# stdstu12/YUME

Hardware: NVIDIA H100
Metric: latent_frames_per_sec (higher is better)
Workload: dtype bf16

## Files before the change

include/yume_b200.h:

```cpp
#ifndef YUME_B200_H_
#define YUME_B200_H_

#ifdef __cplusplus
extern "C" {
#endif

#define YB_OK 0
#define YB_ERR_ARG (-1)
#define YB_ERR_SHAPE (-2)
#define YB_ERR_ALIGNMENT (-3)
#define YB_ERR_NO_DRIVER (-4)
#define YB_ERR_TENSORMAP (-5)
#define YB_ERR_LAUNCH (-6)

int yb_abi_version(void);

#define YB_EPI_BF16 0
#define YB_EPI_GELU_BF16 1
#define YB_EPI_F32 2
#define YB_EPI_GATE_RES 3
#define YB_EPI_RES_BF16 5
#define YB_EPI_GELU_ERF_BF16 4

typedef struct yb_gemm_args {
  unsigned int struct_bytes;
  int cta_pair;
  const void* A;
  const void* B;
  const void* bias;
  void* out;
  const void* gate;
  const void* tok_idx;
  long long lda, ldb, ldo, gate_ld;
  int M, N, K;
  int epilogue;
  int block_n;
  int n_split;
  long long split_stride;
  int a_split;
  long long a_split_stride;
  const void* res;
  long long res_ld;
  int split_k;
  void* ws;
  long long ws_bytes;
} yb_gemm_args;
int yb_gemm_bf16(const yb_gemm_args* args, void* stream);
long long yb_gemm_workspace_bytes(int M, int N, int K, int epilogue, int cta_pair, int split_k);
int yb_gemm_splitk_plan(int tiles, int num_kb, int clusters, int split_k, int* out3);
int yb_gemm_plan(int M, int N, int sms, int* out4);

typedef struct yb_conv3d_args {
  unsigned int struct_bytes;
  int cta_pair;
  const void* xpad;
  const void* w;
  const void* bias;
  void* out;
  const void* res;
  long long ldo, res_ld;
  int T, H, W, Cp, Cout;
  int epilogue;
  int kt, kh, kw;
  int oob_zero_pad;
  int out_t_mul, out_t_add;
  int fuse_w;
  int stride_t, stride_hw;
} yb_conv3d_args;
int yb_conv3d_causal(const yb_conv3d_args* args, void* stream);
int yb_conv3d_plan(int T, int H, int W, int Cout, int kw, int fuse_w, int* out4);

int yb_ln_modulate(const void* x, long long ldx, void* out, long long ldo, int out_f32, const void* scale,
                   const void* shift, long long mod_ld, const void* tok_idx, const void* weight, const void* lnbias,
                   int L, int C, float eps, void* stream);

int yb_rmsnorm_rope(void* qk, long long ld, const void* weight, const void* rope, int rope_len, int L, int C, int D,
                    float eps, void* stream);
int yb_rmsnorm_rope_pieces(void* qk, long long ld, int piece_cols, long long piece_stride, const void* weight,
                           const void* rope, int rope_len, int L, int C, int D, float eps, void* stream);

int yb_qk_norm_rope(void* q, void* k, long long ld, int piece_cols, long long piece_stride, const void* wq, const void* wk,
                    const void* rope, int rope_len, int L, int C, int D, float eps, void* stream);

int yb_attention(const void* q, long long ldq, const void* k, long long ldk, const void* v, long long ldv, void* out,
                 long long ldo, int Lq, int Lk, int heads, float scale, int flags, void* stream);
int yb_attention_ex(const void* q, long long ldq, const void* k, long long ldk, const void* v, long long ldv, void* out,
                    long long ldo, int Lq, int Lk, int heads, float scale, int flags, void* ws, long long ws_bytes,
                    void* trace, void* stream);
#define YB_ATT_P_SMEM 1
#define YB_ATT_EMU_SHIFT 2
#define YB_ATT_ACCUMULATE 2
#define YB_ATT_SPLIT_SHIFT 4
int yb_attention_plan(int Lq, int Lk, int heads, int sms, int flags, int* out4);
long long yb_attention_workspace_bytes(int Lq, int Lk, int heads, int sms, int flags);
int yb_debug_force_split(int ns);
int yb_sp_scatter_qkv(const void* qkv, long long ld, const void* wq, const void* wk, const void* rope, int rope_len,
                      int L, int C, int D, float eps, void* const* peers, int world, int rank, int Lp, void* stream);
int yb_gemm_sp_qkv(const void* A, long long lda, const void* W, const void* bias, int Lp_rows, int C, int K, void* const* peers,
                   int world, int rank, int Lp, void* sums, void* stream);
int yb_sp_bcast_sums(void* local_sums, void* const* peer_tables, int world, int rank, int Lp, void* stream);
int yb_sp_post_norm_rope(void* buf, const void* sums, const void* wq, const void* wk, const void* rope, int rope_len, int L,
                         int Wh, int C, int D, float eps, void* stream);
int yb_attention_sp(const void* q, long long ldq, const void* k, long long ldk, const void* v, long long ldv,
                    void* const* out_peers, long long ldo, int Lq, int Lk, int heads, float scale, int world, int rank,
                    int Lp, int flags, void* ws, long long ws_bytes, void* stream);

int yb_patchify(const void* x, long long sc, long long sf, long long sh, long long sw, void* out, long long ldo,
                int Cin, int F, int H, int W, int ph, int pw, void* stream);

int yb_unpatchify(const void* y, long long ldy, void* out, int Cout, int F, int Hp, int Wp, int ph, int pw,
                  void* stream);

int yb_bcast_add(const void* a, const void* b, void* out, int R1, int R2, int n, void* stream);

int yb_sinusoidal(const void* t, void* out, int n, int dim, void* stream);

int yb_linear_f32_small(const void* in, const void* W, const void* bias, void* out, int M, int N, int K, int silu_in,
                        void* stream);

int yb_linear_f32(const void* in, long long ldi, const void* W, const void* bias, void* out, long long ldo, int M,
                  int N, int K, void* stream);

int yb_gn_stats(const void* x, long long ld, void* stats, long long N, int C, int G, void* stream);
int yb_vae_pad_act(const void* x, long long ldx, int Ts, int Hs, int Ws, int C, void* out, int Cp, int pad, int ft, int fh,
                   int fw, const void* stats, const void* gamma, const void* beta, int G, float eps, int silu,
                   void* stream);
int yb_masked_softmax(const void* S, long long ldS, void* P, long long ldP, int L, int hw, void* stream);
int yb_nchw_to_nhwc_bf16(const void* x, void* out, long long N, int Cn, int ldo, void* stream);
int yb_nhwc_to_nchw_f32(const void* x, long long ldx, void* out, long long N, int Cn, void* stream);
int yb_nhwc_to_nchw_f32_clamp(const void* x, long long ldx, void* out, long long N, int Cn, float lo, float hi, void* stream);
int yb_blend(const void* a, void* b, long long outer, int ea, int eb, int ext, long long inner, void* stream);

int yb_vae_assemble_tiles(const void* const* tile_ptrs, const int* th, const int* tw, const int* tlen, const int* tf0, int nt,
                          int ni, int nj, int C, int F, int H, int W, int row_limit, int blend_extent, int t_limit,
                          int t_blend_extent, void* out, void* stream);

int yb_vae_rms_act(const void* x, long long ldx, void* out, const void* gamma, int T, int Hs, int Ws, int C, int Cp, int up,
                   int silu, void* stream);
int yb_vae_dupup_add(void* main_, const void* x, int Ts, int Hs, int Ws, int in_c, int out_c, int ft, int fs, void* stream);
int yb_vae_unpatchify2_clamp(const void* y, long long ldy, void* out, int T, int H, int W, void* stream);
int yb_vae_avgdown_add(void* main_, const void* x, int T, int H, int W, int in_c, int out_c, int ft, int fs, void* stream);
int yb_vae_patchify2_bf16(const void* video, void* out, long long ldo, int T, int H, int W, void* stream);

int yb_umma_probe(const void* A, const void* B, void* D, int mode, void* stream);

#ifdef __cplusplus
}
#endif
#endif
```

yume_b200/_lib.py:

```python
from __future__ import annotations

import ctypes as C
from pathlib import Path

_LIB_PATH = Path(__file__).resolve().parent / "csrc" / "libyume_b200.so"

YB_EPI_BF16, YB_EPI_GELU_BF16, YB_EPI_F32, YB_EPI_GATE_RES, YB_EPI_GELU_ERF_BF16, YB_EPI_RES_BF16 = 0, 1, 2, 3, 4, 5
YB_ATT_P_SMEM, YB_ATT_ACCUMULATE = 1, 2
ABI_VERSION = 4
YB_ATT_EMU_SHIFT, YB_ATT_SPLIT_SHIFT = 2, 4

_ERRORS = {
    -1: "YB_ERR_ARG (null pointer / bad enum / non-positive size)",
    -2: "YB_ERR_SHAPE (shape not supported by the kernel)",
    -3: "YB_ERR_ALIGNMENT (pointer or stride not 16-byte aligned)",
    -4: "YB_ERR_NO_DRIVER (cuTensorMapEncodeTiled unavailable: no CUDA driver)",
    -5: "YB_ERR_TENSORMAP (driver rejected a TMA descriptor)",
    -6: "YB_ERR_LAUNCH (kernel launch failed)",
}


class YumeB200Error(RuntimeError):
    pass


class GemmArgs(C.Structure):

    _fields_ = [
        ("struct_bytes", C.c_uint), ("cta_pair", C.c_int),
        ("A", C.c_void_p), ("B", C.c_void_p), ("bias", C.c_void_p), ("out", C.c_void_p),
        ("gate", C.c_void_p), ("tok_idx", C.c_void_p),
        ("lda", C.c_longlong), ("ldb", C.c_longlong), ("ldo", C.c_longlong), ("gate_ld", C.c_longlong),
        ("M", C.c_int), ("N", C.c_int), ("K", C.c_int), ("epilogue", C.c_int), ("block_n", C.c_int),
        ("n_split", C.c_int), ("split_stride", C.c_longlong), ("a_split", C.c_int), ("a_split_stride", C.c_longlong),
        ("res", C.c_void_p), ("res_ld", C.c_longlong),
        ("split_k", C.c_int), ("ws", C.c_void_p), ("ws_bytes", C.c_longlong),
    ]


class Conv3dArgs(C.Structure):

    _fields_ = [
        ("struct_bytes", C.c_uint), ("cta_pair", C.c_int),
        ("xpad", C.c_void_p), ("w", C.c_void_p), ("bias", C.c_void_p), ("out", C.c_void_p), ("res", C.c_void_p),
        ("ldo", C.c_longlong), ("res_ld", C.c_longlong),
        ("T", C.c_int), ("H", C.c_int), ("W", C.c_int), ("Cp", C.c_int), ("Cout", C.c_int), ("epilogue", C.c_int),
        ("kt", C.c_int), ("kh", C.c_int), ("kw", C.c_int), ("oob_zero_pad", C.c_int), ("out_t_mul", C.c_int),
        ("out_t_add", C.c_int), ("fuse_w", C.c_int), ("stride_t", C.c_int), ("stride_hw", C.c_int),
    ]


_vp, _ll, _i, _f = C.c_void_p, C.c_longlong, C.c_int, C.c_float
SIGNATURES = {
    "yb_abi_version": (_i, []),
    "yb_gemm_bf16": (_i, [C.POINTER(GemmArgs), _vp]),
    "yb_conv3d_causal": (_i, [C.POINTER(Conv3dArgs), _vp]),
    "yb_gn_stats": (_i, [_vp, _ll, _vp, _ll, _i, _i, _vp]),
    "yb_vae_pad_act": (_i, [_vp, _ll, _i, _i, _i, _i, _vp, _i, _i, _i, _i, _i, _vp, _vp, _vp, _i, _f, _i, _vp]),
    "yb_masked_softmax": (_i, [_vp, _ll, _vp, _ll, _i, _i, _vp]),
    "yb_nchw_to_nhwc_bf16": (_i, [_vp, _vp, _ll, _i, _i, _vp]),
    "yb_nhwc_to_nchw_f32": (_i, [_vp, _ll, _vp, _ll, _i, _vp]),
    "yb_gemm_plan": (_i, [_i, _i, _i, C.POINTER(C.c_int)]),
    "yb_gemm_workspace_bytes": (_ll, [_i, _i, _i, _i, _i, _i]),
    "yb_gemm_splitk_plan": (_i, [_i, _i, _i, _i, C.POINTER(C.c_int)]),
    "yb_conv3d_plan": (_i, [_i, _i, _i, _i, _i, _i, C.POINTER(C.c_int)]),
    "yb_attention_plan": (_i, [_i, _i, _i, _i, _i, C.POINTER(C.c_int)]),
    "yb_nhwc_to_nchw_f32_clamp": (_i, [_vp, _ll, _vp, _ll, _i, C.c_float, C.c_float, _vp]),
    "yb_blend": (_i, [_vp, _vp, _ll, _i, _i, _i, _ll, _vp]),
    "yb_vae_assemble_tiles": (_i, [_vp, _vp, _vp, _vp, _vp, _i, _i, _i, _i, _i, _i, _i, _i, _i, _i, _i, _vp, _vp]),
    "yb_vae_rms_act": (_i, [_vp, _ll, _vp, _vp, _i, _i, _i, _i, _i, _i, _i, _vp]),
    "yb_vae_dupup_add": (_i, [_vp, _vp, _i, _i, _i, _i, _i, _i, _i, _vp]),
    "yb_vae_unpatchify2_clamp": (_i, [_vp, _ll, _vp, _i, _i, _i, _vp]),
    "yb_vae_avgdown_add": (_i, [_vp, _vp, _i, _i, _i, _i, _i, _i, _i, _vp]),
    "yb_vae_patchify2_bf16": (_i, [_vp, _vp, _ll, _i, _i, _i, _vp]),
    "yb_ln_modulate": (_i, [_vp, _ll, _vp, _ll, _i, _vp, _vp, _ll, _vp, _vp, _vp, _i, _i, _f, _vp]),
    "yb_rmsnorm_rope": (_i, [_vp, _ll, _vp, _vp, _i, _i, _i, _i, _f, _vp]),
    "yb_rmsnorm_rope_pieces": (_i, [_vp, _ll, _i, _ll, _vp, _vp, _i, _i, _i, _i, _f, _vp]),
    "yb_qk_norm_rope": (_i, [_vp, _vp, _ll, _i, _ll, _vp, _vp, _vp, _i, _i, _i, _i, _f, _vp]),
    "yb_attention": (_i, [_vp, _ll, _vp, _ll, _vp, _ll, _vp, _ll, _i, _i, _i, _f, _i, _vp]),
    "yb_attention_ex": (_i, [_vp, _ll, _vp, _ll, _vp, _ll, _vp, _ll, _i, _i, _i, _f, _i, _vp, _ll, _vp, _vp]),
    "yb_attention_workspace_bytes": (_ll, [_i, _i, _i, _i, _i]),
    "yb_debug_force_split": (_i, [_i]),
    "yb_sp_scatter_qkv": (_i, [_vp, _ll, _vp, _vp, _vp, _i, _i, _i, _i, _f, C.POINTER(C.c_void_p), _i, _i, _i, _vp]),
    "yb_gemm_sp_qkv": (_i, [_vp, _ll, _vp, _vp, _i, _i, _i, C.POINTER(C.c_void_p), _i, _i, _i, _vp, _vp]),
    "yb_sp_bcast_sums": (_i, [_vp, C.POINTER(C.c_void_p), _i, _i, _i, _vp]),
    "yb_sp_post_norm_rope": (_i, [_vp, _vp, _vp, _vp, _vp, _i, _i, _i, _i, _i, _f, _vp]),
    "yb_attention_sp": (_i, [_vp, _ll, _vp, _ll, _vp, _ll, C.POINTER(C.c_void_p), _ll, _i, _i, _i, _f, _i, _i, _i, _i, _vp, _ll,
                             _vp]),
    "yb_patchify": (_i, [_vp, _ll, _ll, _ll, _ll, _vp, _ll, _i, _i, _i, _i, _i, _i, _vp]),
    "yb_bcast_add": (_i, [_vp, _vp, _vp, _i, _i, _i, _vp]),
    "yb_unpatchify": (_i, [_vp, _ll, _vp, _i, _i, _i, _i, _i, _i, _vp]),
    "yb_sinusoidal": (_i, [_vp, _vp, _i, _i, _vp]),
    "yb_linear_f32_small": (_i, [_vp, _vp, _vp, _vp, _i, _i, _i, _i, _vp]),
    "yb_linear_f32": (_i, [_vp, _ll, _vp, _vp, _vp, _ll, _i, _i, _i, _vp]),
    "yb_umma_probe": (_i, [_vp, _vp, _vp, _i, _vp]),
}

CLIP_SIGNATURES = {
    "yb_resize_bicubic_normalize": (_i, [_vp, _ll, _ll, _ll, _i, _i, _i, _vp, _i, _vp, _vp, _vp]),
}

T5_SIGNATURES = {
    "yb_t5_attention": (_i, [_vp, _ll, _vp, _ll, _vp, _ll, _vp, _ll, _i, _i, _i, _vp, _vp, _vp]),
    "yb_t5_rmsnorm": (_i, [_vp, _ll, _vp, _ll, _i, _vp, _i, _i, _f, _vp]),
    "yb_t5_geglu": (_i, [_vp, _ll, _vp, _ll, _i, _i, _vp]),
}

STREAM_SIGNATURES = {
    "yb_conv3d_causal_hist": (_i, [C.POINTER(Conv3dArgs), _i, _vp]),
    "yb_vae_dupup_add_cont": (_i, [_vp, _vp, _i, _i, _i, _i, _i, _i, _i, _vp]),
    "yb_vae_unpatchify2_clamp_win": (_i, [_vp, _ll, _vp, _ll, _i, _i, _i, _vp]),
    "yb_nhwc_to_nchw_f32_clamp_win": (_i, [_vp, _ll, _vp, _ll, _ll, _i, _f, _f, _vp]),
    "yb_vae_patchify2_bf16_win": (_i, [_vp, _ll, _vp, _ll, _i, _i, _i, _vp]),
    "yb_nchw_to_nhwc_bf16_win": (_i, [_vp, _ll, _vp, _ll, _i, _i, _vp]),
}

YB_EPI_GELU_FP8 = 8


class GemmFp8Args(C.Structure):

    _fields_ = [
        ("struct_bytes", C.c_uint), ("M", C.c_int), ("N", C.c_int), ("K", C.c_int),
        ("A", C.c_void_p), ("a_scale", C.c_void_p), ("B", C.c_void_p), ("b_scale", C.c_void_p), ("bias", C.c_void_p),
        ("out", C.c_void_p), ("out_scale", C.c_void_p), ("gate", C.c_void_p), ("tok_idx", C.c_void_p),
        ("lda", C.c_longlong), ("lds", C.c_longlong), ("ldb", C.c_longlong), ("ldo", C.c_longlong), ("ldos", C.c_longlong),
        ("gate_ld", C.c_longlong), ("epilogue", C.c_int), ("block_n", C.c_int),
    ]


FP8_SIGNATURES = {
    "yb_gemm_fp8": (_i, [C.POINTER(GemmFp8Args), _vp]),
    "yb_ln_modulate_fp8": (_i, [_vp, _ll, _vp, _ll, _vp, _ll, _vp, _vp, _ll, _vp, _vp, _vp, _i, _i, _f, _vp]),
    "yb_quant_rows_fp8": (_i, [_vp, _ll, _vp, _ll, _vp, _ll, _i, _i, _vp]),
}

FP8_ATTN_SIGNATURES = {
    "yb_quant_vt_fp8": (_i, [_vp, _ll, _vp, _vp, _i, _i, _vp]),
    "yb_attention_fp8": (_i, [_vp, _ll, _vp, _ll, _vp, _ll, _vp, _vp, _vp, _ll, _i, _i, _i, _f, _i, _vp, _ll, _vp]),
}

class Conv3dFp8Args(C.Structure):

    _fields_ = [
        ("struct_bytes", C.c_uint), ("x", C.c_void_p), ("x_scale", C.c_void_p), ("w", C.c_void_p), ("w_scale", C.c_void_p),
        ("bias", C.c_void_p), ("out", C.c_void_p), ("res", C.c_void_p), ("ldo", C.c_longlong), ("res_ld", C.c_longlong),
        ("T", C.c_int), ("H", C.c_int), ("W", C.c_int), ("Cp", C.c_int), ("Cout", C.c_int),
        ("kt", C.c_int), ("kh", C.c_int), ("kw", C.c_int), ("t_hist", C.c_int), ("epilogue", C.c_int),
    ]


FP8_VAE_SIGNATURES = {
    "yb_conv3d_fp8": (_i, [C.POINTER(Conv3dFp8Args), _vp]),
    "yb_vae_rms_act_fp8": (_i, [_vp, _ll, _vp, _vp, _vp, _i, _i, _i, _i, _i, _i, _i, _vp]),
}

_lib = None


def lib_path() -> Path:
    return _LIB_PATH


def load():
    global _lib
    if _lib is not None:
        return _lib
    if not _LIB_PATH.exists():
        raise YumeB200Error(
            f"{_LIB_PATH} is missing: build it with `python -m yume_b200.build` (or __graft_entry__.build()). "
            "yume_b200 has no fallback path.")
    lib = C.CDLL(str(_LIB_PATH))
    if lib.yb_abi_version() != ABI_VERSION:
        raise YumeB200Error(f"{_LIB_PATH} has ABI version {lib.yb_abi_version()}, this binding expects {ABI_VERSION}: rebuild it "
                            "(python -m yume_b200.build --force)")
    for name, (res, args) in {**SIGNATURES, **CLIP_SIGNATURES, **T5_SIGNATURES, **STREAM_SIGNATURES,
                              **FP8_SIGNATURES, **FP8_ATTN_SIGNATURES, **FP8_VAE_SIGNATURES}.items():
        fn = getattr(lib, name)
        fn.restype = res
        fn.argtypes = args
    _lib = lib
    return lib


def check(rc: int, what: str) -> None:
    if rc != 0:
        raise YumeB200Error(f"{what} failed: {_ERRORS.get(rc, rc)}")
```

yume_b200/csrc/gemm.cu:

```cuda
#include "yb_host.h"
#include "../../include/yume_b200_stream.h"
#include "yb_ptx.cuh"

namespace yb {

constexpr int GEMM_BLOCK_M = 128;
constexpr int GEMM_BLOCK_K = 64;
constexpr int GEMM_THREADS = 384;
constexpr int GEMM_GROUP_N = 8;
constexpr int GEMM_MAX_STAGES = 8;
constexpr int GEMM_SMEM_BYTES = 227 * 1024;
constexpr int GEMM_A_BYTES = GEMM_BLOCK_M * GEMM_BLOCK_K * 2;
constexpr int GEMM_EPI_STAGE_BYTES = 8 * 16 * 36 * 4;
constexpr int GEMM_EPI_BOX_BYTES = 64 * 128;
constexpr int GEMM_EPI_TMA_BYTES = 2 * 2 * GEMM_EPI_BOX_BYTES;

struct GemmParams {
  int M, N, K;
  const float* bias;
  void* out;
  long long ldo;
  const float* gate;
  long long gate_ld;
  const int* tok_idx;
  int a_split;
  int n_split;
  long long split_stride;
  const __nv_bfloat16* res;
  long long res_ld;
  int conv, cin_chunks;
  int TW, TH, TT, tiles_w, tiles_h;
  int cT, cH, cW;
  int kh, kw;
  int off_t, off_h, off_w;
  int out_t_mul, out_t_add;
  int st_t, st_h, st_w;
  int num_m_tiles, num_n_tiles;
  int block_n, stages;
  int sk_full, sk_ns, sk_per;
  float* sk_ws;
  int tma_out;
  __nv_bfloat16* sp_peers[8];
  float* sp_sums;
  int sp_rank, sp_Lp, sp_Wh, sp_C;
};
constexpr int YB_EPI_SP_QKV = 6;

constexpr int CONVW_ROWS = GEMM_BLOCK_M + 2;
constexpr int CONVW_A_SLAB = 17 * 1024;
constexpr int CONVW_A_STAGES = 4;

__host__ __device__ constexpr int gemm_b_bytes(int block_n) { return ((block_n + 63) / 64) * 64 * GEMM_BLOCK_K * 2; }
__host__ __device__ constexpr int gemm_stage_bytes(int block_n, int convw) { return (convw ? 0 : GEMM_A_BYTES) + gemm_b_bytes(block_n); }
__host__ __device__ constexpr int gemm_a_ring_bytes(int convw) { return convw ? CONVW_A_STAGES * CONVW_A_SLAB : 0; }
__host__ __device__ constexpr bool gemm_has_tma_epilogue(int epi, int convw, int cluster) {
  return cluster == 1 && !convw && (epi == YB_EPI_BF16 || epi == YB_EPI_GELU_BF16 || epi == YB_EPI_GELU_ERF_BF16 ||
                                    epi == YB_EPI_F32 || epi == YB_EPI_GATE_RES);
}
__host__ __device__ constexpr bool gemm_tma_epilogue_only(int epi, int convw, int cluster) {
  return gemm_has_tma_epilogue(epi, convw, cluster) && epi != YB_EPI_BF16 && epi != YB_EPI_F32;
}
__host__ __device__ constexpr int gemm_epi_bytes(bool tma) { return tma ? GEMM_EPI_TMA_BYTES : GEMM_EPI_STAGE_BYTES; }
static int gemm_stages(int block_n, int convw, int epi_bytes) {
  const int s = (GEMM_SMEM_BYTES - 1024 - 256 - epi_bytes - gemm_a_ring_bytes(convw)) / gemm_stage_bytes(block_n, convw);
  return s > GEMM_MAX_STAGES ? GEMM_MAX_STAGES : s;
}

__device__ __forceinline__ void tile_coords(int tile, int num_m_tiles, int num_n_tiles, int& m_tile, int& n_tile) {
  const int per_group = GEMM_GROUP_N * num_m_tiles;
  const int g = tile / per_group;
  const int r = tile - g * per_group;
  const int n_first = g * GEMM_GROUP_N;
  const int n_in_group = min(GEMM_GROUP_N, num_n_tiles - n_first);
  m_tile = r / n_in_group;
  n_tile = n_first + (r - m_tile * n_in_group);
}

template <int EPI>
__device__ __forceinline__ void epilogue_rows16(const GemmParams& p, int col0, int my_row, int my_tok, const float* stage, int lane,
                                                float* sq) {
  constexpr bool kBf16Out = (EPI == YB_EPI_BF16 || EPI == YB_EPI_GELU_BF16 || EPI == YB_EPI_GELU_ERF_BF16 ||
                             EPI == YB_EPI_RES_BF16 || EPI == YB_EPI_SP_QKV);
  if (col0 >= p.N) return;
  if (kBf16Out) {
    const int cq = (lane & 3) * 8;
    float b[8] = {0.f, 0.f, 0.f, 0.f, 0.f, 0.f, 0.f, 0.f};
    if (p.bias) {
      const float4 b0 = __ldg(reinterpret_cast<const float4*>(p.bias + col0 + cq));
      const float4 b1 = __ldg(reinterpret_cast<const float4*>(p.bias + col0 + cq + 4));
      b[0] = b0.x; b[1] = b0.y; b[2] = b0.z; b[3] = b0.w; b[4] = b1.x; b[5] = b1.y; b[6] = b1.z; b[7] = b1.w;
    }
    long long col_off = col0 + cq;
    if (p.n_split > 0) col_off = static_cast<long long>(col0 / p.n_split) * p.split_stride + (col0 % p.n_split) + cq;
    __nv_bfloat16* obase = reinterpret_cast<__nv_bfloat16*>(p.out) + col_off;
    long long ld = p.ldo;
    if (EPI == YB_EPI_SP_QKV) {
      const int part = col0 / p.sp_C, cin = col0 - part * p.sp_C;
      const int peer = cin / p.sp_Wh;
      ld = 3LL * p.sp_Wh;
      obase = p.sp_peers[peer] + static_cast<long long>(p.sp_rank) * p.sp_Lp * ld + part * p.sp_Wh + (cin - peer * p.sp_Wh) + cq;
    }
    uint4 resv[2];
    if (EPI == YB_EPI_RES_BF16) {
#pragma unroll
      for (int it = 0; it < 2; ++it) {
        const int rowi = __shfl_sync(0xffffffffu, my_row, it * 8 + (lane >> 2));
        resv[it] = make_uint4(0u, 0u, 0u, 0u);
        if (rowi >= 0) resv[it] = *reinterpret_cast<const uint4*>(p.res + static_cast<long long>(rowi) * p.res_ld + col0 + cq);
      }
    }
#pragma unroll
    for (int it = 0; it < 2; ++it) {
      const int rr = it * 8 + (lane >> 2);
      const int rowi = __shfl_sync(0xffffffffu, my_row, rr);
      const float4 a0 = *reinterpret_cast<const float4*>(stage + rr * 36 + cq);
      const float4 a1 = *reinterpret_cast<const float4*>(stage + rr * 36 + cq + 4);
      float v[8] = {a0.x + b[0], a0.y + b[1], a0.z + b[2], a0.w + b[3], a1.x + b[4], a1.y + b[5], a1.z + b[6], a1.w + b[7]};
      if (EPI == YB_EPI_GELU_BF16) {
#pragma unroll
        for (int i = 0; i < 8; ++i) v[i] = gelu_tanh(v[i]);
      }
      if (EPI == YB_EPI_GELU_ERF_BF16) {
#pragma unroll
        for (int i = 0; i < 8; ++i) v[i] = 0.5f * v[i] * (1.0f + erff(v[i] * 0.7071067811865476f));
      }
      if (EPI == YB_EPI_RES_BF16) {
        const __nv_bfloat162* rh = reinterpret_cast<const __nv_bfloat162*>(&resv[it]);
#pragma unroll
        for (int i = 0; i < 4; ++i) {
          const float2 f = __bfloat1622float2(rh[i]);
          v[2 * i] += f.x;
          v[2 * i + 1] += f.y;
        }
      }
      if (rowi >= 0) {
        uint4 w;
        w.x = pack_bf16x2(v[0], v[1]);
        w.y = pack_bf16x2(v[2], v[3]);
        w.z = pack_bf16x2(v[4], v[5]);
        w.w = pack_bf16x2(v[6], v[7]);
        *reinterpret_cast<uint4*>(obase + static_cast<long long>(rowi) * ld) = w;
        if (EPI == YB_EPI_SP_QKV) {
          const __nv_bfloat162* wh = reinterpret_cast<const __nv_bfloat162*>(&w);
          float acc = 0.f;
#pragma unroll
          for (int i = 0; i < 4; ++i) {
            const float2 f = __bfloat1622float2(wh[i]);
            acc += f.x * f.x + f.y * f.y;
          }
          sq[it] += acc;
        }
      }
    }
  } else {
    const int cq = (lane & 7) * 4;
    float4 b = make_float4(0.f, 0.f, 0.f, 0.f);
    if (p.bias) b = __ldg(reinterpret_cast<const float4*>(p.bias + col0 + cq));
    float* obase = reinterpret_cast<float*>(p.out) + col0 + cq;
    float4 xv[4], gv[4];
    int rowv[4];
#pragma unroll
    for (int it = 0; it < 4; ++it) {
      const int rr = it * 4 + (lane >> 3);
      const int tok = __shfl_sync(0xffffffffu, my_tok, rr);
      rowv[it] = __shfl_sync(0xffffffffu, my_row, rr);
      xv[it] = make_float4(0.f, 0.f, 0.f, 0.f);
      gv[it] = make_float4(1.f, 1.f, 1.f, 1.f);
      if (EPI == YB_EPI_GATE_RES && rowv[it] >= 0) {
        xv[it] = *reinterpret_cast<const float4*>(obase + static_cast<long long>(rowv[it]) * p.ldo);
        if (p.gate) gv[it] = __ldg(reinterpret_cast<const float4*>(p.gate + static_cast<long long>(tok) * p.gate_ld + col0 + cq));
      }
    }
#pragma unroll
    for (int it = 0; it < 4; ++it) {
      const int rr = it * 4 + (lane >> 3);
      float4 a = *reinterpret_cast<const float4*>(stage + rr * 36 + cq);
      a.x += b.x; a.y += b.y; a.z += b.z; a.w += b.w;
      if (rowv[it] >= 0) {
        float4* o4 = reinterpret_cast<float4*>(obase + static_cast<long long>(rowv[it]) * p.ldo);
        if (EPI == YB_EPI_F32) {
          *o4 = a;
        } else {
          float4 x = xv[it];
          x.x += a.x * gv[it].x; x.y += a.y * gv[it].y; x.z += a.z * gv[it].z; x.w += a.w * gv[it].w;
          *o4 = x;
        }
      }
    }
  }
}

template <int EPI, int NM>
__device__ __forceinline__ void epilogue_tma(const GemmParams& p, const CUtensorMap* tmO, const float (&acc)[128], uint8_t* bufs,
                                             int row0, int col0, int wg, int wtid, uint32_t& nbox) {
  constexpr bool kF32 = (EPI == YB_EPI_F32 || EPI == YB_EPI_GATE_RES);
  constexpr int BOX_COLS = kF32 ? 32 : 64;
  constexpr int GROUPS = BOX_COLS / 8;
  if (row0 >= p.M) return;
  const int lane = wtid & 31;
  const int r = (wtid >> 5) * 16 + (lane >> 2);
  const int sw = lane >> 2, c2 = 2 * (lane & 3);
  const int ncols = min(NM, p.N - col0);
  const float* g_lo = nullptr;
  const float* g_hi = nullptr;
  if (EPI == YB_EPI_GATE_RES && p.gate != nullptr) {
    int t_lo = 0, t_hi = 0;
    if (p.tok_idx != nullptr) {
      if (row0 + r < p.M) t_lo = p.tok_idx[row0 + r];
      if (row0 + r + 8 < p.M) t_hi = p.tok_idx[row0 + r + 8];
    }
    g_lo = p.gate + static_cast<long long>(t_lo) * p.gate_ld;
    g_hi = p.gate + static_cast<long long>(t_hi) * p.gate_ld;
  }
#pragma unroll
  for (int s = 0; s < NM / BOX_COLS; ++s) {
    if (s * BOX_COLS < ncols) {
      uint8_t* buf = bufs + (nbox & 1) * GEMM_EPI_BOX_BYTES;
      if (wtid == 0) bulk_wait_read<1>();
      named_bar_sync(1 + wg, 128);
#pragma unroll
      for (int j = 0; j < GROUPS; ++j) {
        const int g = s * GROUPS + j;
        const int col = col0 + s * BOX_COLS + 8 * j + c2;
        float2 b = make_float2(0.f, 0.f);
        const bool in = s * BOX_COLS + 8 * j < ncols;
        if (p.bias && in) b = __ldg(reinterpret_cast<const float2*>(p.bias + col));
        float2 lo = make_float2(acc[4 * g] + b.x, acc[4 * g + 1] + b.y);
        float2 hi = make_float2(acc[4 * g + 2] + b.x, acc[4 * g + 3] + b.y);
        if (EPI == YB_EPI_GELU_BF16) {
          lo = make_float2(gelu_tanh(lo.x), gelu_tanh(lo.y));
          hi = make_float2(gelu_tanh(hi.x), gelu_tanh(hi.y));
        }
        if (EPI == YB_EPI_GELU_ERF_BF16) {
          auto ge = [](float v) { return 0.5f * v * (1.0f + erff(v * 0.7071067811865476f)); };
          lo = make_float2(ge(lo.x), ge(lo.y));
          hi = make_float2(ge(hi.x), ge(hi.y));
        }
        if (EPI == YB_EPI_GATE_RES && g_lo != nullptr && in) {
          const float2 gl = __ldg(reinterpret_cast<const float2*>(g_lo + col));
          const float2 gh = __ldg(reinterpret_cast<const float2*>(g_hi + col));
          lo = make_float2(lo.x * gl.x, lo.y * gl.y);
          hi = make_float2(hi.x * gh.x, hi.y * gh.y);
        }
        if (kF32) {
          const int off = (((2 * j + ((lane & 3) >> 1)) ^ sw) << 4) + 8 * (lane & 1);
          *reinterpret_cast<float2*>(buf + r * 128 + off) = lo;
          *reinterpret_cast<float2*>(buf + (r + 8) * 128 + off) = hi;
        } else {
          const int off = ((j ^ sw) << 4) + 4 * (lane & 3);
          *reinterpret_cast<uint32_t*>(buf + r * 128 + off) = pack_bf16x2(lo.x, lo.y);
          *reinterpret_cast<uint32_t*>(buf + (r + 8) * 128 + off) = pack_bf16x2(hi.x, hi.y);
        }
      }
      fence_proxy_async_smem();
      named_bar_sync(1 + wg, 128);
      if (wtid == 0) {
        if (EPI == YB_EPI_GATE_RES) tma_reduce_add_2d(tmO, buf, col0 + s * BOX_COLS, row0);
        else tma_store_2d(tmO, buf, col0 + s * BOX_COLS, row0);
        bulk_commit();
      }
      ++nbox;
    }
  }
}

template <int NM>
__device__ __forceinline__ void gemm_mma_k64(float (&acc)[128], uint32_t sa, uint32_t sb, int block_n, bool zero_first) {
  const uint64_t ad0 = make_smem_desc_sw128(sa, 16, 1024), bd0 = make_smem_desc_sw128(sb, 16, 1024);
  const int nb64 = (block_n + 63) >> 6;
#pragma unroll
  for (int k = 0; k < GEMM_BLOCK_K / 16; ++k) {
    const uint64_t ad = ad0 + 2 * k, bd = bd0 + 2 * k;
    const uint32_t accum = (zero_first && k == 0) ? 0u : 1u;
    if (NM == 256) {
      wgmma_ss_n256<0>(acc, ad, bd, accum);
    } else if (NM == 128) {
      wgmma_ss_n128<0>(acc, ad, bd, accum);
    } else {
      wgmma_ss_n64<0>(acc, ad, bd, accum);
      if (nb64 > 1) wgmma_ss_n64<32>(acc, ad, bd + (8192 >> 4), accum);
      if (nb64 > 2) wgmma_ss_n64<64>(acc, ad, bd + (16384 >> 4), accum);
      if (nb64 > 3) wgmma_ss_n64<96>(acc, ad, bd + (24576 >> 4), accum);
    }
  }
}

template <int CLUSTER>
__device__ __forceinline__ void release_slot(uint64_t* bar, int lane) {
  __syncwarp();
  if (lane == 0) {
    if (CLUSTER == 1) {
      mbar_arrive(bar);
    } else {
      mbar_arrive_cluster(bar, 0);
      mbar_arrive_cluster(bar, 1);
    }
  }
}

template <int EPI, int CONVW, int CLUSTER, int NM>
__global__ void __launch_bounds__(GEMM_THREADS, 1)
gemm_kernel(const __grid_constant__ CUtensorMap tmA, const __grid_constant__ CUtensorMap tmB, const __grid_constant__ CUtensorMap tmO,
            const GemmParams p) {
  static_assert(!(CONVW && CLUSTER != 1), "the kw-fused conv runs on single CTAs");
  constexpr bool kTmaEpi = gemm_has_tma_epilogue(EPI, CONVW, CLUSTER);
  const bool tma_out = gemm_tma_epilogue_only(EPI, CONVW, CLUSTER) || (kTmaEpi && p.tma_out);
  extern __shared__ uint8_t smem_raw[];
  uint8_t* smem = reinterpret_cast<uint8_t*>((reinterpret_cast<uintptr_t>(smem_raw) + 1023) & ~uintptr_t(1023));
  const int block_n = p.block_n, stages = p.stages;
  const int stage_bytes = gemm_stage_bytes(block_n, CONVW);
  uint8_t* a_ring = smem + stages * stage_bytes;
  float* epi = reinterpret_cast<float*>(a_ring + gemm_a_ring_bytes(CONVW));
  uint64_t* full_bar = reinterpret_cast<uint64_t*>(reinterpret_cast<uint8_t*>(epi) + gemm_epi_bytes(kTmaEpi));
  uint64_t* empty_bar = full_bar + GEMM_MAX_STAGES;
  uint64_t* a_full = empty_bar + GEMM_MAX_STAGES;
  uint64_t* a_empty = a_full + CONVW_A_STAGES;

  const int warp = threadIdx.x >> 5, lane = threadIdx.x & 31;
  const int rank = CLUSTER == 2 ? static_cast<int>(cluster_ctarank()) : 0;
  const int tile_first = blockIdx.x / CLUSTER, tile_step = gridDim.x / CLUSTER;
  const int num_tiles = p.num_m_tiles * p.num_n_tiles;
  const int num_kb = (p.K + GEMM_BLOCK_K - 1) / GEMM_BLOCK_K;
  const int num_work = p.sk_full + (num_tiles - p.sk_full) * p.sk_ns;
  auto decode_work = [&](int w, int& tile, int& kb0, int& kb1, int& part) {
    tile = w; kb0 = 0; kb1 = num_kb; part = -1;
    if (w >= p.sk_full) {
      const int u = w - p.sk_full;
      tile = p.sk_full + u / p.sk_ns;
      kb0 = (u % p.sk_ns) * p.sk_per;
      kb1 = min(num_kb, kb0 + p.sk_per);
      part = u;
    }
  };
  auto conv_box = [&](int mt, int& it, int& ih, int& iw) {
    const int per_t = p.tiles_h * p.tiles_w;
    it = mt / per_t;
    const int rem = mt - it * per_t;
    ih = rem / p.tiles_w;
    iw = rem - ih * p.tiles_w;
  };

  if (threadIdx.x == 0) {
    tma_prefetch_desc(&tmA);
    tma_prefetch_desc(&tmB);
    if (tma_out) tma_prefetch_desc(&tmO);
    for (int i = 0; i < stages; ++i) {
      mbar_init(&full_bar[i], 1);
      mbar_init(&empty_bar[i], 8 * CLUSTER);
    }
    for (int i = 0; i < (CONVW ? CONVW_A_STAGES : 0); ++i) {
      mbar_init(&a_full[i], 1);
      mbar_init(&a_empty[i], 8);
    }
    fence_barrier_init();
  }
  __syncthreads();
  if (CLUSTER > 1) cluster_sync_all();

  if (warp < 4) {
    setmaxnreg_dec<40>();
    if (warp == 0 && lane == 0) {
      int stage = 0, a_stage = 0;
      uint32_t phase = 0, a_phase = 0;
      for (int w = tile_first; w < num_work; w += tile_step) {
        int tile, kb0, kb1, part, m_tile, n_tile;
        decode_work(w, tile, kb0, kb1, part);
        tile_coords(tile, p.num_m_tiles, p.num_n_tiles, m_tile, n_tile);
        if (CONVW) {
          int it, ih, iw;
          conv_box(m_tile, it, ih, iw);
          const int groups = num_kb / 3;
          for (int g = 0; g < groups; ++g) {
            const int tdh = g / p.cin_chunks, cc = g - tdh * p.cin_chunks;
            const int dt = tdh / p.kh, dh = tdh - dt * p.kh;
            mbar_wait(&a_empty[a_stage], a_phase ^ 1);
            mbar_arrive_expect_tx(&a_full[a_stage], CONVW_ROWS * GEMM_BLOCK_K * 2);
            tma_load_4d(a_ring + a_stage * CONVW_A_SLAB, &tmA, &a_full[a_stage], cc * GEMM_BLOCK_K, iw * GEMM_BLOCK_M - p.off_w,
                        ih + dh - p.off_h, it + dt - p.off_t);
            if (++a_stage == CONVW_A_STAGES) {
              a_stage = 0;
              a_phase ^= 1;
            }
#pragma unroll 1
            for (int dw = 0; dw < 3; ++dw) {
              mbar_wait(&empty_bar[stage], phase ^ 1);
              mbar_arrive_expect_tx(&full_bar[stage], block_n * GEMM_BLOCK_K * 2);
              tma_load_2d(smem + stage * stage_bytes, &tmB, &full_bar[stage], ((tdh * 3 + dw) * p.cin_chunks + cc) * GEMM_BLOCK_K,
                          n_tile * block_n);
              if (++stage == stages) {
                stage = 0;
                phase ^= 1;
              }
            }
          }
          continue;
        }
        for (int kb = kb0; kb < kb1; ++kb) {
          if (CLUSTER > 1) mbar_wait_cluster(&empty_bar[stage], phase ^ 1);
          else mbar_wait(&empty_bar[stage], phase ^ 1);
          uint8_t* sa = smem + stage * stage_bytes;
          uint8_t* sb = sa + GEMM_A_BYTES;
          mbar_arrive_expect_tx(&full_bar[stage], GEMM_A_BYTES + block_n * GEMM_BLOCK_K * 2);
          const int kcol = kb * GEMM_BLOCK_K;
          const int mt = m_tile * CLUSTER + rank;
          if (p.conv) {
            const int tap = kb / p.cin_chunks, cc = kb - tap * p.cin_chunks;
            const int dt = tap / (p.kh * p.kw), dh = (tap / p.kw) % p.kh, dw = tap % p.kw;
            int it, ih, iw;
            conv_box(mt, it, ih, iw);
            tma_load_4d(sa, &tmA, &full_bar[stage], cc * GEMM_BLOCK_K, iw * p.TW * p.st_w + dw - p.off_w,
                        ih * p.TH * p.st_h + dh - p.off_h, it * p.TT * p.st_t + dt - p.off_t);
          } else {
            const int chunk = kcol / p.a_split;
            tma_load_3d(sa, &tmA, &full_bar[stage], kcol - chunk * p.a_split, mt * GEMM_BLOCK_M, chunk);
          }
          if (CLUSTER == 1) {
            tma_load_2d(sb, &tmB, &full_bar[stage], kcol, n_tile * block_n);
          } else {
            const int half = block_n / 2;
            tma_load_2d_multicast(sb + rank * half * GEMM_BLOCK_K * 2, &tmB, &full_bar[stage], kcol, n_tile * block_n + rank * half,
                                  static_cast<uint16_t>(3));
          }
          if (++stage == stages) {
            stage = 0;
            phase ^= 1;
          }
        }
      }
    }
  } else {
    setmaxnreg_inc<232>();
    const int wg = (warp >> 2) - 1;
    const int r0 = wg * 64 + (warp & 3) * 16;
    float* stage_buf = epi + (warp - 4) * (16 * 36);
    uint8_t* box_bufs = reinterpret_cast<uint8_t*>(epi) + wg * 2 * GEMM_EPI_BOX_BYTES;
    uint32_t nbox = 0;
    int stage = 0, a_stage = 0;
    uint32_t phase = 0, a_phase = 0;
    float acc[128];
#pragma unroll
    for (int i = 0; i < 128; ++i) acc[i] = 0.f;
    for (int w = tile_first; w < num_work; w += tile_step) {
      int tile, kb0, kb1, part, m_tile, n_tile;
      decode_work(w, tile, kb0, kb1, part);
      tile_coords(tile, p.num_m_tiles, p.num_n_tiles, m_tile, n_tile);
      const int mt = m_tile * CLUSTER + rank;
      int my_row = -1;
      if (!tma_out) {
        const int r = r0 + (lane & 15);
        if (p.conv) {
          int it, ih, iw;
          conv_box(mt, it, ih, iw);
          const int tw = r % p.TW, th = (r / p.TW) % p.TH, tt = r / (p.TW * p.TH);
          const int t = it * p.TT + tt, h = ih * p.TH + th, ww = iw * p.TW + tw;
          my_row = (t < p.cT && h < p.cH && ww < p.cW) ? ((t * p.out_t_mul + p.out_t_add) * p.cH + h) * p.cW + ww : -1;
        } else {
          const int row = mt * GEMM_BLOCK_M + r;
          my_row = row < p.M ? row : -1;
        }
      }
      if (EPI == YB_EPI_GATE_RES && part < 0 && my_row >= 0 && lane < 16) {
        const char* xrow = reinterpret_cast<const char*>(reinterpret_cast<const float*>(p.out) +
                                                         static_cast<long long>(my_row) * p.ldo + n_tile * block_n);
        const int ncols = min(block_n, p.N - n_tile * block_n);
        for (int b = 0; b < ncols * 4; b += 128) asm volatile("prefetch.global.L2 [%0];" ::"l"(xrow + b));
      }
      int prev = -1;
      if (CONVW) {
        int prev_a = -1;
        const int groups = num_kb / 3;
        for (int g = 0; g < groups; ++g) {
          mbar_wait(&a_full[a_stage], a_phase);
          const uint32_t sa = smem_u32(a_ring + a_stage * CONVW_A_SLAB) + wg * 64 * 128;
#pragma unroll 1
          for (int dw = 0; dw < 3; ++dw) {
            mbar_wait(&full_bar[stage], phase);
            fence_regs(acc);
            wgmma_fence();
            gemm_mma_k64<NM>(acc, sa + dw * 128, smem_u32(smem + stage * stage_bytes), block_n, g == 0 && dw == 0);
            wgmma_commit();
            wgmma_wait<1>();
            fence_regs(acc);
            if (prev >= 0) release_slot<1>(&empty_bar[prev], lane);
            if (dw == 0 && prev_a >= 0) {
              release_slot<1>(&a_empty[prev_a], lane);
              prev_a = -1;
            }
            prev = stage;
            if (++stage == stages) {
              stage = 0;
              phase ^= 1;
            }
          }
          prev_a = a_stage;
          if (++a_stage == CONVW_A_STAGES) {
            a_stage = 0;
            a_phase ^= 1;
          }
        }
        wgmma_wait<0>();
        fence_regs(acc);
        if (prev >= 0) release_slot<1>(&empty_bar[prev], lane);
        if (prev_a >= 0) release_slot<1>(&a_empty[prev_a], lane);
      } else {
        for (int kb = kb0; kb < kb1; ++kb) {
          mbar_wait(&full_bar[stage], phase);
          const uint32_t sa = smem_u32(smem + stage * stage_bytes);
          fence_regs(acc);
          wgmma_fence();
          gemm_mma_k64<NM>(acc, sa + wg * 64 * 128, sa + GEMM_A_BYTES, block_n, kb == kb0);
          wgmma_commit();
          wgmma_wait<1>();
          fence_regs(acc);
          if (prev >= 0) release_slot<CLUSTER>(&empty_bar[prev], lane);
          prev = stage;
          if (++stage == stages) {
            stage = 0;
            phase ^= 1;
          }
        }
        wgmma_wait<0>();
        fence_regs(acc);
        if (prev >= 0) release_slot<CLUSTER>(&empty_bar[prev], lane);
      }

      const int q4 = lane >> 2, c2 = 2 * (lane & 3);
      if (part >= 0) {
        float* wbase = p.sk_ws + (static_cast<long long>(part) * 256 + rank * GEMM_BLOCK_M + r0) * block_n;
#pragma unroll
        for (int g = 0; g < 32; ++g) {
          if (g * 8 < block_n) {
            *reinterpret_cast<float2*>(wbase + q4 * block_n + g * 8 + c2) = make_float2(acc[4 * g], acc[4 * g + 1]);
            *reinterpret_cast<float2*>(wbase + (q4 + 8) * block_n + g * 8 + c2) = make_float2(acc[4 * g + 2], acc[4 * g + 3]);
          }
        }
        continue;
      }
      if (tma_out) {
        epilogue_tma<EPI, NM>(p, &tmO, acc, box_bufs, mt * GEMM_BLOCK_M + wg * 64, n_tile * block_n, wg, threadIdx.x & 127, nbox);
        continue;
      }
      int my_tok = 0;
      if (EPI == YB_EPI_GATE_RES && p.gate != nullptr && p.tok_idx != nullptr && my_row >= 0) my_tok = p.tok_idx[my_row];
      float sq[2] = {0.f, 0.f};
      auto flush_sq = [&](int part_) {
#pragma unroll
        for (int it = 0; it < 2; ++it) {
          float v = sq[it];
          v += __shfl_xor_sync(0xffffffffu, v, 1);
          v += __shfl_xor_sync(0xffffffffu, v, 2);
          const int rowi = __shfl_sync(0xffffffffu, my_row, it * 8 + (lane >> 2));
          if ((lane & 3) == 0 && rowi >= 0 && part_ < 2) atomicAdd(p.sp_sums + rowi * 2 + part_, v);
          sq[it] = 0.f;
        }
      };
      int cur_part = (EPI == YB_EPI_SP_QKV) ? (n_tile * block_n) / p.sp_C : 0;
#pragma unroll
      for (int c = 0; c < 8; ++c) {
        if (c * 32 < block_n) {
#pragma unroll
          for (int g = 0; g < 4; ++g) {
            const int i = 4 * (4 * c + g);
            *reinterpret_cast<float2*>(stage_buf + q4 * 36 + g * 8 + c2) = make_float2(acc[i], acc[i + 1]);
            *reinterpret_cast<float2*>(stage_buf + (q4 + 8) * 36 + g * 8 + c2) = make_float2(acc[i + 2], acc[i + 3]);
          }
          __syncwarp();
          const int col0 = n_tile * block_n + c * 32;
          if (EPI == YB_EPI_SP_QKV && col0 < p.N) {
            const int pt = col0 / p.sp_C;
            if (pt != cur_part) {
              flush_sq(cur_part);
              cur_part = pt;
            }
          }
          epilogue_rows16<EPI>(p, col0, my_row, my_tok, stage_buf, lane, sq);
          __syncwarp();
        }
      }
      if (EPI == YB_EPI_SP_QKV) flush_sq(cur_part);
    }
    if (tma_out && (threadIdx.x & 127) == 0) bulk_wait<0>();
  }
  if (CLUSTER > 1) cluster_sync_all();
}

__global__ void __launch_bounds__(256) gemm_splitk_combine_kernel(const GemmParams p, int tail_tiles) {
  const int block_n = p.block_n, quads = block_n >> 2;
  const long long total = static_cast<long long>(tail_tiles) * 256 * quads;
  for (long long i = blockIdx.x * static_cast<long long>(blockDim.x) + threadIdx.x; i < total;
       i += static_cast<long long>(gridDim.x) * blockDim.x) {
    const int cq = static_cast<int>(i % quads) * 4;
    const long long rr = i / quads;
    const int r = static_cast<int>(rr & 255);
    const int t = static_cast<int>(rr >> 8);
    int m_tile, n_tile;
    tile_coords(p.sk_full + t, p.num_m_tiles, p.num_n_tiles, m_tile, n_tile);
    const int row = m_tile * 256 + r, col = n_tile * block_n + cq;
    if (row >= p.M || col >= p.N) continue;
    float4 a = make_float4(0.f, 0.f, 0.f, 0.f);
    for (int sg = 0; sg < p.sk_ns; ++sg) {
      const float4 v = *reinterpret_cast<const float4*>(p.sk_ws + ((static_cast<long long>(t) * p.sk_ns + sg) * 256 + r) * block_n + cq);
      a.x += v.x; a.y += v.y; a.z += v.z; a.w += v.w;
    }
    if (p.bias) {
      const float4 b = __ldg(reinterpret_cast<const float4*>(p.bias + col));
      a.x += b.x; a.y += b.y; a.z += b.z; a.w += b.w;
    }
    float4 g = make_float4(1.f, 1.f, 1.f, 1.f);
    if (p.gate) {
      const long long tok = p.tok_idx ? p.tok_idx[row] : 0;
      g = __ldg(reinterpret_cast<const float4*>(p.gate + tok * p.gate_ld + col));
    }
    float4* xp = reinterpret_cast<float4*>(reinterpret_cast<float*>(p.out) + static_cast<long long>(row) * p.ldo + col);
    float4 x = *xp;
    x.x += a.x * g.x; x.y += a.y * g.y; x.z += a.z * g.z; x.w += a.w * g.w;
    *xp = x;
  }
}

static void gemm_splitk_plan(int tiles, int num_kb, int clusters, int force_ns, int* full, int* ns, int* per) {
  *full = tiles; *ns = 1; *per = num_kb;
  if (clusters <= 0 || force_ns == 1) return;
  int r = tiles % clusters;
  if (force_ns >= 2) {
    if (num_kb < 2 * force_ns) return;
    if (tiles <= clusters || r == 0) r = tiles < clusters ? tiles : clusters;
    *ns = force_ns;
  } else {
    if (tiles <= clusters || r == 0) return;
    double best = 0.85;
    for (int n = 2; n <= 12 && num_kb / n >= 8; ++n) {
      const int pr = (num_kb + n - 1) / n;
      const double cost = static_cast<double>((r * n + clusters - 1) / clusters) * (pr + 5.0) / num_kb + 6.0 / num_kb + 0.01 * n;
      if (cost < best) { best = cost; *ns = n; }
    }
    if (*ns == 1) return;
  }
  *per = (num_kb + *ns - 1) / *ns;
  while (*ns > 1 && (*ns - 1) * *per >= num_kb) --*ns;
  if (*ns == 1) { *per = num_kb; return; }
  *full = tiles - r;
}

static int pair_block_n(int M, int N, int clusters) {
  (void)M;
  (void)clusters;
  return N >= 256 ? 256 : ((N + 31) / 32) * 32;
}

template <typename Kern>
static int pair_max_clusters(Kern kern) {
  cudaLaunchConfig_t cfg = {};
  cfg.gridDim = dim3(2 * (sm_count() / 2));
  cfg.blockDim = dim3(GEMM_THREADS);
  cfg.dynamicSmemBytes = GEMM_SMEM_BYTES;
  cudaLaunchAttribute attr;
  attr.id = cudaLaunchAttributeClusterDimension;
  attr.val.clusterDim.x = 2;
  attr.val.clusterDim.y = 1;
  attr.val.clusterDim.z = 1;
  cfg.attrs = &attr;
  cfg.numAttrs = 1;
  int n = 0;
  if (cudaOccupancyMaxActiveClusters(&n, kern, &cfg) != cudaSuccess || n <= 0) {
    (void)cudaGetLastError();
    n = sm_count() / 2;
  }
  return n;
}

template <int EPI, int CONVW, int CLUSTER>
static int launch_gemm(const CUtensorMap& tmA, const CUtensorMap& tmB, const CUtensorMap* tmO, GemmParams& p, cudaStream_t stream,
                       int split_k = 1, void* ws = nullptr, long long ws_bytes = 0) {
  static const CUtensorMap no_map = {};
  if (gemm_tma_epilogue_only(EPI, CONVW, CLUSTER) && tmO == nullptr) return YB_ERR_ARG;
  p.tma_out = gemm_has_tma_epilogue(EPI, CONVW, CLUSTER) && tmO != nullptr;
  if (!p.tma_out) tmO = &no_map;
  const int nm = p.block_n == 256 ? 2 : p.block_n == 128 ? 1 : 0;
  if (CLUSTER == 1 && nm == 0) return YB_ERR_ARG;
  auto kern = nm == 2 ? gemm_kernel<EPI, CONVW, CLUSTER, 256> : nm == 1 ? gemm_kernel<EPI, CONVW, CLUSTER, 128>
                      : gemm_kernel<EPI, CONVW, CLUSTER, CLUSTER == 1 ? 128 : 64>;
  static bool attr_set[3][kMaxDevices] = {};
  if (int rc = ensure_dynamic_smem(kern, GEMM_SMEM_BYTES, attr_set[nm], "gemm")) return rc;
  if (CLUSTER == 2) p.num_m_tiles = p.conv ? (p.num_m_tiles + 1) / 2 : (p.M + 255) / 256;
  else if (!p.conv) p.num_m_tiles = (p.M + GEMM_BLOCK_M - 1) / GEMM_BLOCK_M;
  p.num_n_tiles = (p.N + p.block_n - 1) / p.block_n;
  p.stages = gemm_stages(p.block_n, CONVW, gemm_epi_bytes(gemm_has_tma_epilogue(EPI, CONVW, CLUSTER)));
  const int tiles = p.num_m_tiles * p.num_n_tiles;
  static int max_clusters[kMaxDevices] = {0};
  const int dev = current_device();
  if (max_clusters[dev] == 0) max_clusters[dev] = CLUSTER == 2 ? pair_max_clusters(kern) : sm_count();
  p.sk_full = tiles; p.sk_ns = 1; p.sk_per = 0; p.sk_ws = nullptr;
  int tail = 0;
  if (CLUSTER == 2 && EPI == YB_EPI_GATE_RES && !p.conv && ws != nullptr && split_k != 1) {
    const int num_kb = (p.K + GEMM_BLOCK_K - 1) / GEMM_BLOCK_K;
    gemm_splitk_plan(tiles, num_kb, max_clusters[dev], split_k, &p.sk_full, &p.sk_ns, &p.sk_per);
    tail = tiles - p.sk_full;
    const long long need = static_cast<long long>(tail) * p.sk_ns * 256 * p.block_n * 4;
    if (tail > 0 && (ws_bytes < need || (reinterpret_cast<uintptr_t>(ws) & 0xF))) {
      p.sk_full = tiles; p.sk_ns = 1; tail = 0;
    }
    if (tail > 0) p.sk_ws = static_cast<float*>(ws);
  }
  const int work = p.sk_full + tail * p.sk_ns;
  const int groups = work < max_clusters[dev] ? work : max_clusters[dev];
  cudaLaunchConfig_t cfg = {};
  cfg.gridDim = dim3(groups * CLUSTER);
  cfg.blockDim = dim3(GEMM_THREADS);
  cfg.dynamicSmemBytes = GEMM_SMEM_BYTES;
  cfg.stream = stream;
  cudaLaunchAttribute attr;
  attr.id = cudaLaunchAttributeClusterDimension;
  attr.val.clusterDim.x = CLUSTER;
  attr.val.clusterDim.y = 1;
  attr.val.clusterDim.z = 1;
  cfg.attrs = &attr;
  cfg.numAttrs = 1;
  (void)cudaLaunchKernelEx(&cfg, kern, tmA, tmB, *tmO, p);
  int rc = check_launch("gemm");
  if (rc || tail == 0) return rc;
  const long long total = static_cast<long long>(tail) * 256 * (p.block_n / 4);
  gemm_splitk_combine_kernel<<<static_cast<int>((total + 255) / 256), 256, 0, stream>>>(p, tail);
  return check_launch("gemm_splitk_combine");
}

static void conv_plan(int T, int H, int W, int block_n, int kw, int fuse_policy, int* TW, int* TH, int* TT, bool* fused) {
  auto pow2_ge = [](int v) { int p = 1; while (p < v) p <<= 1; return p; };
  double best = -1.0;
  const double vox = static_cast<double>(T) * H * W;
  for (int tw = 128; tw >= 1; tw >>= 1) {
    if (tw > pow2_ge(W)) continue;
    for (int th = 128 / tw; th >= 1; th >>= 1) {
      const int tt = 128 / (tw * th);
      const double tiles = static_cast<double>((W + tw - 1) / tw) * ((H + th - 1) / th) * ((T + tt - 1) / tt);
      const double util = vox / (tiles * 128.0);
      if (util > best + 1e-9) { best = util; *TW = tw; *TH = th; *TT = tt; }
    }
  }
  *fused = false;
  if (kw == 3 && fuse_policy != 1 && (W >= 64 || fuse_policy == 2)) {
    const double util128 = static_cast<double>(W) / (((W + 127) / 128) * 128.0);
    *fused = fuse_policy == 2 || util128 >= (block_n == 128 ? 0.70 : 0.95) * best;
  }
  if (*fused) { *TW = 128; *TH = 1; *TT = 1; }
}

}

extern "C" int yb_gemm_sp_qkv(const void* A, long long lda, const void* W, const void* bias, int Lp_rows, int C, int K,
                              void* const* peers, int world, int rank, int Lp, void* sums, void* stream_) {
  using namespace yb;
  if (!A || !W || !peers || !sums || Lp_rows <= 0 || C <= 0 || K <= 0) return YB_ERR_ARG;
  if (world < 2 || world > 8 || rank < 0 || rank >= world || Lp < Lp_rows) return YB_ERR_ARG;
  if (C % (world * 128) != 0 || K % 8 != 0 || (lda % 8)) return YB_ERR_SHAPE;
  GemmParams p = {};
  p.M = Lp_rows;
  p.N = 3 * C;
  p.K = K;
  p.bias = static_cast<const float*>(bias);
  p.out = peers[rank];
  p.ldo = 3LL * (C / world);
  p.a_split = K;
  p.sp_rank = rank;
  p.sp_Lp = Lp;
  p.sp_Wh = C / world;
  p.sp_C = C;
  p.sp_sums = static_cast<float*>(sums);
  for (int i = 0; i < 8; ++i) p.sp_peers[i] = i < world ? static_cast<__nv_bfloat16*>(peers[i]) : nullptr;
  p.block_n = pair_block_n(p.M, p.N, sm_count() / 2);
  CUtensorMap tmA, tmB;
  int rc = make_tmap_bf16_3d(&tmA, A, 1, p.M, K, lda, lda * (long long)p.M + 8, GEMM_BLOCK_M, GEMM_BLOCK_K);
  if (rc) return rc;
  rc = make_tmap_bf16_2d(&tmB, W, p.N, K, K, p.block_n / 2, GEMM_BLOCK_K);
  if (rc) return rc;
  return launch_gemm<YB_EPI_SP_QKV, 0, 2>(tmA, tmB, nullptr, p, reinterpret_cast<cudaStream_t>(stream_));
}

extern "C" int yb_gemm_plan(int M, int N, int sms, int* out4) {
  if (M <= 0 || N <= 0 || sms < 2 || !out4) return YB_ERR_ARG;
  out4[0] = 0;
  out4[1] = (N % 256 == 0 || N > 1024) ? 256 : 128;
  out4[2] = (M + yb::GEMM_BLOCK_M - 1) / yb::GEMM_BLOCK_M;
  out4[3] = (N + out4[1] - 1) / out4[1];
  return YB_OK;
}

extern "C" int yb_conv3d_plan(int T, int H, int W, int Cout, int kw, int fuse_w, int* out4) {
  if (T <= 0 || H <= 0 || W <= 0 || Cout <= 0 || (kw != 1 && kw != 3) || fuse_w < 0 || fuse_w > 2 || !out4) return YB_ERR_ARG;
  bool fused = false;
  yb::conv_plan(T, H, W, (Cout % 256 == 0) ? 256 : 128, kw, fuse_w, &out4[0], &out4[1], &out4[2], &fused);
  out4[3] = fused ? 1 : 0;
  return YB_OK;
}

extern "C" int yb_gemm_splitk_plan(int tiles, int num_kb, int clusters, int split_k, int* out3) {
  if (tiles <= 0 || num_kb <= 0 || clusters <= 0 || split_k < 0 || split_k > 12 || !out3) return YB_ERR_ARG;
  yb::gemm_splitk_plan(tiles, num_kb, clusters, split_k, &out3[0], &out3[1], &out3[2]);
  return YB_OK;
}

extern "C" long long yb_gemm_workspace_bytes(int M, int N, int K, int epilogue, int cta_pair, int split_k) {
  using namespace yb;
  if (M <= 0 || N <= 0 || K <= 0 || epilogue != YB_EPI_GATE_RES || split_k == 1 || split_k < 0 || split_k > 12) return 0;
  if (cta_pair != 2) return 0;
  static int max_clusters[kMaxDevices] = {0};
  static bool attr_set[kMaxDevices] = {false};
  const int dev = current_device();
  if (max_clusters[dev] == 0) {
    if (ensure_dynamic_smem(gemm_kernel<YB_EPI_GATE_RES, 0, 2, 256>, GEMM_SMEM_BYTES, attr_set, "gemm")) return 0;
    max_clusters[dev] = pair_max_clusters(gemm_kernel<YB_EPI_GATE_RES, 0, 2, 256>);
  }
  const int bn = pair_block_n(M, N, max_clusters[dev]);
  const int tiles = ((M + 255) / 256) * ((N + bn - 1) / bn);
  int full, ns, per;
  gemm_splitk_plan(tiles, (K + GEMM_BLOCK_K - 1) / GEMM_BLOCK_K, max_clusters[dev], split_k, &full, &ns, &per);
  return static_cast<long long>(tiles - full) * ns * 256 * bn * 4;
}

extern "C" int yb_gemm_bf16(const yb_gemm_args* a, void* stream_) {
  using namespace yb;
  if (!a || !a->A || !a->B || !a->out) return YB_ERR_ARG;
  if (a->M <= 0 || a->N <= 0 || a->K <= 0) return YB_ERR_ARG;
  if (a->N % 32 != 0 || a->K % 8 != 0) return YB_ERR_SHAPE;
  if (a->epilogue < 0 || a->epilogue > YB_EPI_RES_BF16) return YB_ERR_ARG;
  if (a->epilogue == YB_EPI_RES_BF16 && (!a->res || (a->res_ld % 8))) return YB_ERR_ARG;
  if ((a->lda % 8) || (a->ldb % 8) || (a->ldo % 8) || (reinterpret_cast<uintptr_t>(a->out) & 0xF)) return YB_ERR_ALIGNMENT;
  cudaStream_t stream = reinterpret_cast<cudaStream_t>(stream_);
  if (a->struct_bytes != sizeof(yb_gemm_args)) return YB_ERR_ARG;
  if (a->cta_pair < 0 || a->cta_pair > 2 || a->split_k < 0 || a->split_k > 12) return YB_ERR_ARG;
  int a_split = a->K;
  long long a_chunk_ld = 0;
  if (a->a_split > 0) {
    if (a->a_split % GEMM_BLOCK_K != 0 || a->K % a->a_split != 0) return YB_ERR_SHAPE;
    a_split = a->a_split;
    a_chunk_ld = a->a_split_stride;
  }
  const int a_chunks = a->K / a_split;
  if (a->n_split < 0 || (a->n_split > 0 && (a->n_split % 32 != 0 || a->epilogue != YB_EPI_BF16))) return YB_ERR_ARG;
  GemmParams p;
  p.M = a->M;
  p.N = a->N;
  p.K = a->K;
  p.bias = static_cast<const float*>(a->bias);
  p.out = a->out;
  p.ldo = a->ldo;
  p.gate = static_cast<const float*>(a->gate);
  p.gate_ld = a->gate_ld;
  p.tok_idx = static_cast<const int*>(a->tok_idx);
  p.a_split = a_split;
  p.res = static_cast<const __nv_bfloat16*>(a->res);
  p.res_ld = a->res_ld;
  p.conv = 0;
  p.n_split = a->n_split;
  p.split_stride = a->split_stride;
  p.block_n = 0;
  p.stages = 0;
  CUtensorMap tmA, tmB;
  int rc = make_tmap_bf16_3d(&tmA, a->A, a_chunks, a->M, a_split, a->lda, a_chunks > 1 ? a_chunk_ld : a->lda * (long long)a->M + 8,
                             GEMM_BLOCK_M, GEMM_BLOCK_K);
  if (rc) return rc;
  const bool pair = a->cta_pair == 2;
  if (pair) {
    int bn = a->block_n;
    if (bn == 0) bn = pair_block_n(a->M, a->N, sm_count() / 2);
    if (bn < 32 || bn > 256 || bn % 32 != 0) return YB_ERR_ARG;
    p.block_n = bn;
    rc = make_tmap_bf16_2d(&tmB, a->B, a->N, a->K, a->ldb, bn / 2, GEMM_BLOCK_K);
    if (rc) return rc;
    switch (a->epilogue) {
      case YB_EPI_BF16: return launch_gemm<YB_EPI_BF16, 0, 2>(tmA, tmB, nullptr, p, stream);
      case YB_EPI_GELU_BF16: return launch_gemm<YB_EPI_GELU_BF16, 0, 2>(tmA, tmB, nullptr, p, stream);
      case YB_EPI_F32: return launch_gemm<YB_EPI_F32, 0, 2>(tmA, tmB, nullptr, p, stream);
      case YB_EPI_GELU_ERF_BF16: return launch_gemm<YB_EPI_GELU_ERF_BF16, 0, 2>(tmA, tmB, nullptr, p, stream);
      case YB_EPI_RES_BF16: return launch_gemm<YB_EPI_RES_BF16, 0, 2>(tmA, tmB, nullptr, p, stream);
      default: return launch_gemm<YB_EPI_GATE_RES, 0, 2>(tmA, tmB, nullptr, p, stream, a->split_k, a->ws, a->ws_bytes);
    }
  }
  const int block_n = (a->block_n == 128 || a->block_n == 256) ? a->block_n : ((a->N % 256 == 0 || a->N > 1024) ? 256 : 128);
  rc = make_tmap_bf16_2d(&tmB, a->B, a->N, a->K, a->ldb, block_n, GEMM_BLOCK_K);
  if (rc) return rc;
  p.block_n = block_n;
  CUtensorMap tmO;
  const CUtensorMap* tmo = nullptr;
  if (a->n_split == 0 && a->epilogue != YB_EPI_RES_BF16) {
    const int elem = (a->epilogue == YB_EPI_F32 || a->epilogue == YB_EPI_GATE_RES) ? 4 : 2;
    rc = make_tmap_out_2d(&tmO, a->out, a->M, a->N, a->ldo, elem, 64);
    if (rc) return rc;
    tmo = &tmO;
  }
  switch (a->epilogue) {
    case YB_EPI_BF16: return launch_gemm<YB_EPI_BF16, 0, 1>(tmA, tmB, tmo, p, stream);
    case YB_EPI_GELU_BF16: return launch_gemm<YB_EPI_GELU_BF16, 0, 1>(tmA, tmB, tmo, p, stream);
    case YB_EPI_F32: return launch_gemm<YB_EPI_F32, 0, 1>(tmA, tmB, tmo, p, stream);
    case YB_EPI_GELU_ERF_BF16: return launch_gemm<YB_EPI_GELU_ERF_BF16, 0, 1>(tmA, tmB, tmo, p, stream);
    case YB_EPI_RES_BF16: return launch_gemm<YB_EPI_RES_BF16, 0, 1>(tmA, tmB, nullptr, p, stream);
    default: return launch_gemm<YB_EPI_GATE_RES, 0, 1>(tmA, tmB, tmo, p, stream);
  }
}


static int conv3d_launch(const yb_conv3d_args* a, int t_hist, void* stream_) {
  using namespace yb;
  if (!a || !a->xpad || !a->w || !a->out) return YB_ERR_ARG;
  if (a->struct_bytes != sizeof(yb_conv3d_args)) return YB_ERR_ARG;
  if (a->T <= 0 || a->H <= 0 || a->W <= 0 || a->Cp <= 0 || a->Cout <= 0) return YB_ERR_ARG;
  if (t_hist < 0) return YB_ERR_ARG;
  if (a->Cp % 64 != 0 || a->Cout % 32 != 0) return YB_ERR_SHAPE;
  if ((a->ldo % 8) || (reinterpret_cast<uintptr_t>(a->out) & 0xF)) return YB_ERR_ALIGNMENT;
  if (a->epilogue != YB_EPI_BF16 && a->epilogue != YB_EPI_F32 && a->epilogue != YB_EPI_RES_BF16) return YB_ERR_ARG;
  if (a->epilogue == YB_EPI_RES_BF16 && (!a->res || (a->res_ld % 8))) return YB_ERR_ARG;
  cudaStream_t stream = reinterpret_cast<cudaStream_t>(stream_);
  GemmParams p;
  const int kt = a->kt > 0 ? a->kt : 3, kh = a->kh > 0 ? a->kh : 3, kw = a->kw > 0 ? a->kw : 3;
  if ((kt != 1 && kt != 3) || (kh != 1 && kh != 3) || (kw != 1 && kw != 3)) return YB_ERR_SHAPE;
  const int block_n = (a->Cout % 256 == 0) ? 256 : 128;
  bool fuse_w = false;
  if (a->cta_pair < 0 || a->cta_pair > 2) return YB_ERR_ARG;
  const int st_t = a->stride_t > 0 ? a->stride_t : 1, st_hw = a->stride_hw > 0 ? a->stride_hw : 1;
  if (st_t > 2 || st_hw > 2) return YB_ERR_ARG;
  const bool strided = st_t > 1 || st_hw > 1;
  if (strided && !a->oob_zero_pad) return YB_ERR_ARG;
  if (t_hist > 0 && (!a->oob_zero_pad || t_hist != (st_t > 1 ? 1 : kt - 1))) return YB_ERR_ARG;
  const int inT = a->T + t_hist;
  int oT = a->T, oH = a->H, oW = a->W;
  if (st_t > 1) oT = (inT - kt) / st_t + 1;
  if (st_hw > 1) { oH = (a->H + 1 - kh) / st_hw + 1; oW = (a->W + 1 - kw) / st_hw + 1; }
  if (oT <= 0 || oH <= 0 || oW <= 0) return YB_ERR_SHAPE;
  const bool conv_pair = a->cta_pair == 1;
  conv_plan(oT, oH, oW, block_n, kw, (conv_pair || strided) ? 1 : a->fuse_w, &p.TW, &p.TH, &p.TT, &fuse_w);
  p.tiles_w = (oW + p.TW - 1) / p.TW;
  p.tiles_h = (oH + p.TH - 1) / p.TH;
  const int tiles_t = (oT + p.TT - 1) / p.TT;
  const int taps = kt * kh * kw;
  p.conv = fuse_w ? 2 : 1;
  p.cin_chunks = a->Cp / 64;
  p.cT = oT; p.cH = oH; p.cW = oW;
  p.kh = kh; p.kw = kw;
  p.st_t = st_t; p.st_h = st_hw; p.st_w = st_hw;
  p.off_t = (a->oob_zero_pad && st_t == 1) ? kt - 1 - t_hist : 0;
  p.off_h = (a->oob_zero_pad && st_hw == 1) ? kh / 2 : 0;
  p.off_w = (a->oob_zero_pad && st_hw == 1) ? kw / 2 : 0;
  p.out_t_mul = a->out_t_mul > 0 ? a->out_t_mul : 1;
  p.out_t_add = a->out_t_add;
  p.M = oT * oH * oW;
  p.N = a->Cout;
  p.K = taps * a->Cp;
  p.num_m_tiles = tiles_t * p.tiles_h * p.tiles_w;
  p.bias = static_cast<const float*>(a->bias);
  p.out = a->out;
  p.ldo = a->ldo;
  p.gate = nullptr; p.gate_ld = 0; p.tok_idx = nullptr;
  p.a_split = p.K; p.n_split = 0; p.split_stride = 0;
  p.res = static_cast<const __nv_bfloat16*>(a->res);
  p.res_ld = a->res_ld;
  CUtensorMap tmA, tmB;
  const int padT = a->oob_zero_pad ? 0 : kt - 1, padH = a->oob_zero_pad ? 0 : kh - 1, padW = a->oob_zero_pad ? 0 : kw - 1;
  int rc = make_tmap_bf16_4d(&tmA, a->xpad, inT + padT, a->H + padH, a->W + padW, a->Cp, p.TT, p.TH,
                             fuse_w ? CONVW_ROWS : p.TW, 64, st_t, st_hw, st_hw);
  if (rc) return rc;
  rc = make_tmap_bf16_2d(&tmB, a->w, a->Cout, static_cast<uint64_t>(taps) * a->Cp, static_cast<uint64_t>(taps) * a->Cp,
                         block_n, GEMM_BLOCK_K);
  if (rc) return rc;
  if (conv_pair && !fuse_w) {
    p.conv = 1;
    p.block_n = a->Cout <= 256 ? a->Cout : (a->Cout % 192 == 0 ? 192 : 256);
    CUtensorMap tmBp;
    rc = make_tmap_bf16_2d(&tmBp, a->w, a->Cout, static_cast<uint64_t>(taps) * a->Cp, static_cast<uint64_t>(taps) * a->Cp,
                           p.block_n / 2, GEMM_BLOCK_K);
    if (rc) return rc;
    switch (a->epilogue) {
      case YB_EPI_BF16: return launch_gemm<YB_EPI_BF16, 0, 2>(tmA, tmBp, nullptr, p, stream);
      case YB_EPI_F32: return launch_gemm<YB_EPI_F32, 0, 2>(tmA, tmBp, nullptr, p, stream);
      default: return launch_gemm<YB_EPI_RES_BF16, 0, 2>(tmA, tmBp, nullptr, p, stream);
    }
  }
  p.block_n = block_n;
#define YB_CONV_DISPATCH(CW)                                                                  \
  switch (a->epilogue) {                                                                     \
    case YB_EPI_BF16: return launch_gemm<YB_EPI_BF16, CW, 1>(tmA, tmB, nullptr, p, stream);   \
    case YB_EPI_F32: return launch_gemm<YB_EPI_F32, CW, 1>(tmA, tmB, nullptr, p, stream);     \
    default: return launch_gemm<YB_EPI_RES_BF16, CW, 1>(tmA, tmB, nullptr, p, stream);        \
  }
  if (fuse_w) {
    YB_CONV_DISPATCH(1)
  } else {
    YB_CONV_DISPATCH(0)
  }
#undef YB_CONV_DISPATCH
}

extern "C" int yb_conv3d_causal(const yb_conv3d_args* a, void* stream) { return conv3d_launch(a, 0, stream); }

extern "C" int yb_conv3d_causal_hist(const yb_conv3d_args* a, int t_hist, void* stream) {
  if (t_hist <= 0) return YB_ERR_ARG;
  return conv3d_launch(a, t_hist, stream);
}
```

yume_b200/csrc/yb_ptx.cuh:

```cuda
#pragma once
#include <cstdint>
#include <cstdio>
#include <cuda.h>
#include <cuda_runtime.h>
#include <cuda_bf16.h>

namespace yb {

__device__ __forceinline__ uint32_t smem_u32(const void* p) {
  return static_cast<uint32_t>(__cvta_generic_to_shared(p));
}

template <int N>
__device__ __forceinline__ void setmaxnreg_inc() {
  asm volatile("setmaxnreg.inc.sync.aligned.u32 %0;\n" ::"n"(N));
}
template <int N>
__device__ __forceinline__ void setmaxnreg_dec() {
  asm volatile("setmaxnreg.dec.sync.aligned.u32 %0;\n" ::"n"(N));
}
__device__ __forceinline__ void named_bar_sync(int id, int count) {
  asm volatile("bar.sync %0, %1;" ::"r"(id), "r"(count) : "memory");
}

__device__ __forceinline__ void mbar_init(uint64_t* bar, uint32_t count) {
  asm volatile("mbarrier.init.shared::cta.b64 [%0], %1;" ::"r"(smem_u32(bar)), "r"(count) : "memory");
}
__device__ __forceinline__ void fence_barrier_init() {
  asm volatile("fence.mbarrier_init.release.cluster;" ::: "memory");
}
__device__ __forceinline__ void fence_proxy_async_smem() {
  asm volatile("fence.proxy.async.shared::cta;" ::: "memory");
}
__device__ __forceinline__ void mbar_arrive_expect_tx(uint64_t* bar, uint32_t bytes) {
  asm volatile("mbarrier.arrive.expect_tx.shared::cta.b64 _, [%0], %1;" ::"r"(smem_u32(bar)), "r"(bytes)
               : "memory");
}
__device__ __forceinline__ void mbar_arrive(uint64_t* bar) {
  asm volatile("mbarrier.arrive.shared::cta.b64 _, [%0];" ::"r"(smem_u32(bar)) : "memory");
}
__device__ __forceinline__ bool mbar_try_wait(uint64_t* bar, uint32_t parity) {
  uint32_t ok;
  asm volatile(
      "{\n\t.reg .pred p;\n\t"
      "mbarrier.try_wait.parity.shared::cta.b64 p, [%1], %2;\n\t"
      "selp.u32 %0, 1, 0, p;\n\t}\n"
      : "=r"(ok)
      : "r"(smem_u32(bar)), "r"(parity)
      : "memory");
  return ok != 0;
}
#ifndef YB_WAIT_LIMIT_CYCLES
#define YB_WAIT_LIMIT_CYCLES 8000000000LL
#endif
__device__ __forceinline__ void mbar_wait(uint64_t* bar, uint32_t parity) {
  if (mbar_try_wait(bar, parity)) return;
  const long long t0 = clock64();
  while (!mbar_try_wait(bar, parity)) {
    if (clock64() - t0 > YB_WAIT_LIMIT_CYCLES) {
#ifdef YB_DEBUG_WAIT
      printf("yb: mbarrier wait timeout block=(%d,%d) thread=%d bar=%u parity=%u\n", blockIdx.x, blockIdx.y,
             threadIdx.x, smem_u32(bar), parity);
#endif
      __trap();
    }
  }
}
__device__ __forceinline__ void mbar_wait_cluster(uint64_t* bar, uint32_t parity) {
  const long long t0 = clock64();
  for (;;) {
    uint32_t ok;
    asm volatile(
        "{\n\t.reg .pred p;\n\t"
        "mbarrier.try_wait.parity.acquire.cluster.shared::cta.b64 p, [%1], %2;\n\t"
        "selp.u32 %0, 1, 0, p;\n\t}\n"
        : "=r"(ok)
        : "r"(smem_u32(bar)), "r"(parity)
        : "memory");
    if (ok) return;
    if (clock64() - t0 > YB_WAIT_LIMIT_CYCLES) __trap();
  }
}

__device__ __forceinline__ uint32_t cluster_ctarank() {
  uint32_t r;
  asm volatile("mov.u32 %0, %%cluster_ctarank;" : "=r"(r));
  return r;
}
__device__ __forceinline__ void cluster_sync_all() {
  asm volatile("barrier.cluster.arrive.release.aligned;\n\tbarrier.cluster.wait.acquire.aligned;" ::: "memory");
}
__device__ __forceinline__ void mbar_arrive_cluster(uint64_t* bar, uint32_t cta) {
  uint32_t remote;
  asm volatile("mapa.shared::cluster.u32 %0, %1, %2;" : "=r"(remote) : "r"(smem_u32(bar)), "r"(cta));
  asm volatile("mbarrier.arrive.release.cluster.shared::cluster.b64 _, [%0];" ::"r"(remote) : "memory");
}

__device__ __forceinline__ void tma_prefetch_desc(const CUtensorMap* tmap) {
  asm volatile("prefetch.tensormap [%0];" ::"l"(reinterpret_cast<uint64_t>(tmap)) : "memory");
}
__device__ __forceinline__ void tma_load_2d(void* smem_dst, const CUtensorMap* tmap, uint64_t* bar, int c0, int c1) {
  asm volatile(
      "cp.async.bulk.tensor.2d.shared::cluster.global.tile.mbarrier::complete_tx::bytes [%0], [%1, {%3, %4}], [%2];"
      ::"r"(smem_u32(smem_dst)), "l"(reinterpret_cast<uint64_t>(tmap)), "r"(smem_u32(bar)), "r"(c0), "r"(c1)
      : "memory");
}
__device__ __forceinline__ void tma_load_2d_multicast(void* smem_dst, const CUtensorMap* tmap, uint64_t* bar, int c0, int c1,
                                                      uint16_t mask) {
  asm volatile(
      "cp.async.bulk.tensor.2d.shared::cluster.global.mbarrier::complete_tx::bytes.multicast::cluster [%0], [%1, {%3, %4}], "
      "[%2], %5;" ::"r"(smem_u32(smem_dst)),
      "l"(reinterpret_cast<uint64_t>(tmap)), "r"(smem_u32(bar)), "r"(c0), "r"(c1), "h"(mask)
      : "memory");
}
__device__ __forceinline__ void tma_load_3d(void* smem_dst, const CUtensorMap* tmap, uint64_t* bar, int c0, int c1,
                                            int c2) {
  asm volatile(
      "cp.async.bulk.tensor.3d.shared::cluster.global.tile.mbarrier::complete_tx::bytes [%0], [%1, {%3, %4, %5}], [%2];"
      ::"r"(smem_u32(smem_dst)), "l"(reinterpret_cast<uint64_t>(tmap)), "r"(smem_u32(bar)), "r"(c0), "r"(c1), "r"(c2)
      : "memory");
}
__device__ __forceinline__ void tma_load_4d(void* smem_dst, const CUtensorMap* tmap, uint64_t* bar, int c0, int c1,
                                            int c2, int c3) {
  asm volatile(
      "cp.async.bulk.tensor.4d.shared::cluster.global.tile.mbarrier::complete_tx::bytes [%0], [%1, {%3, %4, %5, %6}], [%2];"
      ::"r"(smem_u32(smem_dst)), "l"(reinterpret_cast<uint64_t>(tmap)), "r"(smem_u32(bar)), "r"(c0), "r"(c1), "r"(c2),
      "r"(c3)
      : "memory");
}
__device__ __forceinline__ void tma_store_2d(const CUtensorMap* tmap, const void* smem_src, int c0, int c1) {
  asm volatile("cp.async.bulk.tensor.2d.global.shared::cta.bulk_group [%0, {%2, %3}], [%1];"
               ::"l"(reinterpret_cast<uint64_t>(tmap)), "r"(smem_u32(smem_src)), "r"(c0), "r"(c1)
               : "memory");
}
__device__ __forceinline__ void tma_reduce_add_2d(const CUtensorMap* tmap, const void* smem_src, int c0, int c1) {
  asm volatile("cp.reduce.async.bulk.tensor.2d.global.shared::cta.add.tile.bulk_group [%0, {%2, %3}], [%1];"
               ::"l"(reinterpret_cast<uint64_t>(tmap)), "r"(smem_u32(smem_src)), "r"(c0), "r"(c1)
               : "memory");
}
__device__ __forceinline__ void bulk_commit() { asm volatile("cp.async.bulk.commit_group;" ::: "memory"); }
template <int N>
__device__ __forceinline__ void bulk_wait_read() {
  asm volatile("cp.async.bulk.wait_group.read %0;" ::"n"(N) : "memory");
}
template <int N>
__device__ __forceinline__ void bulk_wait() {
  asm volatile("cp.async.bulk.wait_group %0;" ::"n"(N) : "memory");
}

__device__ __forceinline__ uint64_t make_smem_desc_sw128(uint32_t smem_addr, uint32_t lbo_bytes, uint32_t sbo_bytes) {
  uint64_t d = 0;
  d |= static_cast<uint64_t>((smem_addr & 0x3FFFF) >> 4);
  d |= static_cast<uint64_t>((lbo_bytes >> 4) & 0x3FFF) << 16;
  d |= static_cast<uint64_t>((sbo_bytes >> 4) & 0x3FFF) << 32;
  d |= static_cast<uint64_t>(1) << 62;
  return d;
}
__device__ __forceinline__ void wgmma_fence() { asm volatile("wgmma.fence.sync.aligned;" ::: "memory"); }
__device__ __forceinline__ void wgmma_commit() { asm volatile("wgmma.commit_group.sync.aligned;" ::: "memory"); }
template <int N>
__device__ __forceinline__ void wgmma_wait() {
  asm volatile("wgmma.wait_group.sync.aligned %0;" ::"n"(N) : "memory");
}
template <int R>
__device__ __forceinline__ void fence_regs(float (&d)[R]) {
#pragma unroll
  for (int i = 0; i < R; ++i) asm volatile("" : "+f"(d[i])::"memory");
}

template <int OFF>
__device__ __forceinline__ void wgmma_ss_n64(float (&d)[128], uint64_t adesc, uint64_t bdesc, uint32_t accumulate) {
  asm volatile(
      "{\n\t.reg .pred p;\n\t"
      "setp.ne.b32 p, %34, 0;\n\t"
      "wgmma.mma_async.sync.aligned.m64n64k16.f32.bf16.bf16 {%0, %1, %2, %3, %4, %5, %6, %7, %8, %9, %10, %11, %12, %13, %14, %15, %16, %17, %18, %19, %20, %21, %22, %23, %24, %25, %26, %27, %28, %29, %30, %31}, %32, %33, p, 1, 1, 0, 0;\n\t}\n"
      : "+f"(d[OFF + 0]), "+f"(d[OFF + 1]), "+f"(d[OFF + 2]), "+f"(d[OFF + 3]), "+f"(d[OFF + 4]), "+f"(d[OFF + 5]), "+f"(d[OFF + 6]), "+f"(d[OFF + 7]), "+f"(d[OFF + 8]), "+f"(d[OFF + 9]), "+f"(d[OFF + 10]), "+f"(d[OFF + 11]), "+f"(d[OFF + 12]), "+f"(d[OFF + 13]), "+f"(d[OFF + 14]), "+f"(d[OFF + 15]), "+f"(d[OFF + 16]), "+f"(d[OFF + 17]), "+f"(d[OFF + 18]), "+f"(d[OFF + 19]), "+f"(d[OFF + 20]), "+f"(d[OFF + 21]), "+f"(d[OFF + 22]), "+f"(d[OFF + 23]), "+f"(d[OFF + 24]), "+f"(d[OFF + 25]), "+f"(d[OFF + 26]), "+f"(d[OFF + 27]), "+f"(d[OFF + 28]), "+f"(d[OFF + 29]), "+f"(d[OFF + 30]), "+f"(d[OFF + 31])
      : "l"(adesc), "l"(bdesc), "r"(accumulate));
}
template <int OFF>
__device__ __forceinline__ void wgmma_ss_n128(float (&d)[128], uint64_t adesc, uint64_t bdesc, uint32_t accumulate) {
  asm volatile(
      "{\n\t.reg .pred p;\n\t"
      "setp.ne.b32 p, %66, 0;\n\t"
      "wgmma.mma_async.sync.aligned.m64n128k16.f32.bf16.bf16 {%0, %1, %2, %3, %4, %5, %6, %7, %8, %9, %10, %11, %12, %13, %14, %15, %16, %17, %18, %19, %20, %21, %22, %23, %24, %25, %26, %27, %28, %29, %30, %31, %32, %33, %34, %35, %36, %37, %38, %39, %40, %41, %42, %43, %44, %45, %46, %47, %48, %49, %50, %51, %52, %53, %54, %55, %56, %57, %58, %59, %60, %61, %62, %63}, %64, %65, p, 1, 1, 0, 0;\n\t}\n"
      : "+f"(d[OFF + 0]), "+f"(d[OFF + 1]), "+f"(d[OFF + 2]), "+f"(d[OFF + 3]), "+f"(d[OFF + 4]), "+f"(d[OFF + 5]), "+f"(d[OFF + 6]), "+f"(d[OFF + 7]), "+f"(d[OFF + 8]), "+f"(d[OFF + 9]), "+f"(d[OFF + 10]), "+f"(d[OFF + 11]), "+f"(d[OFF + 12]), "+f"(d[OFF + 13]), "+f"(d[OFF + 14]), "+f"(d[OFF + 15]), "+f"(d[OFF + 16]), "+f"(d[OFF + 17]), "+f"(d[OFF + 18]), "+f"(d[OFF + 19]), "+f"(d[OFF + 20]), "+f"(d[OFF + 21]), "+f"(d[OFF + 22]), "+f"(d[OFF + 23]), "+f"(d[OFF + 24]), "+f"(d[OFF + 25]), "+f"(d[OFF + 26]), "+f"(d[OFF + 27]), "+f"(d[OFF + 28]), "+f"(d[OFF + 29]), "+f"(d[OFF + 30]), "+f"(d[OFF + 31]), "+f"(d[OFF + 32]), "+f"(d[OFF + 33]), "+f"(d[OFF + 34]), "+f"(d[OFF + 35]), "+f"(d[OFF + 36]), "+f"(d[OFF + 37]), "+f"(d[OFF + 38]), "+f"(d[OFF + 39]), "+f"(d[OFF + 40]), "+f"(d[OFF + 41]), "+f"(d[OFF + 42]), "+f"(d[OFF + 43]), "+f"(d[OFF + 44]), "+f"(d[OFF + 45]), "+f"(d[OFF + 46]), "+f"(d[OFF + 47]), "+f"(d[OFF + 48]), "+f"(d[OFF + 49]), "+f"(d[OFF + 50]), "+f"(d[OFF + 51]), "+f"(d[OFF + 52]), "+f"(d[OFF + 53]), "+f"(d[OFF + 54]), "+f"(d[OFF + 55]), "+f"(d[OFF + 56]), "+f"(d[OFF + 57]), "+f"(d[OFF + 58]), "+f"(d[OFF + 59]), "+f"(d[OFF + 60]), "+f"(d[OFF + 61]), "+f"(d[OFF + 62]), "+f"(d[OFF + 63])
      : "l"(adesc), "l"(bdesc), "r"(accumulate));
}
template <int OFF>
__device__ __forceinline__ void wgmma_ss_n256(float (&d)[128], uint64_t adesc, uint64_t bdesc, uint32_t accumulate) {
  asm volatile(
      "{\n\t.reg .pred p;\n\t"
      "setp.ne.b32 p, %130, 0;\n\t"
      "wgmma.mma_async.sync.aligned.m64n256k16.f32.bf16.bf16 {%0, %1, %2, %3, %4, %5, %6, %7, %8, %9, %10, %11, %12, %13, %14, %15, %16, %17, %18, %19, %20, %21, %22, %23, %24, %25, %26, %27, %28, %29, %30, %31, %32, %33, %34, %35, %36, %37, %38, %39, %40, %41, %42, %43, %44, %45, %46, %47, %48, %49, %50, %51, %52, %53, %54, %55, %56, %57, %58, %59, %60, %61, %62, %63, %64, %65, %66, %67, %68, %69, %70, %71, %72, %73, %74, %75, %76, %77, %78, %79, %80, %81, %82, %83, %84, %85, %86, %87, %88, %89, %90, %91, %92, %93, %94, %95, %96, %97, %98, %99, %100, %101, %102, %103, %104, %105, %106, %107, %108, %109, %110, %111, %112, %113, %114, %115, %116, %117, %118, %119, %120, %121, %122, %123, %124, %125, %126, %127}, %128, %129, p, 1, 1, 0, 0;\n\t}\n"
      : "+f"(d[OFF + 0]), "+f"(d[OFF + 1]), "+f"(d[OFF + 2]), "+f"(d[OFF + 3]), "+f"(d[OFF + 4]), "+f"(d[OFF + 5]), "+f"(d[OFF + 6]), "+f"(d[OFF + 7]), "+f"(d[OFF + 8]), "+f"(d[OFF + 9]), "+f"(d[OFF + 10]), "+f"(d[OFF + 11]), "+f"(d[OFF + 12]), "+f"(d[OFF + 13]), "+f"(d[OFF + 14]), "+f"(d[OFF + 15]), "+f"(d[OFF + 16]), "+f"(d[OFF + 17]), "+f"(d[OFF + 18]), "+f"(d[OFF + 19]), "+f"(d[OFF + 20]), "+f"(d[OFF + 21]), "+f"(d[OFF + 22]), "+f"(d[OFF + 23]), "+f"(d[OFF + 24]), "+f"(d[OFF + 25]), "+f"(d[OFF + 26]), "+f"(d[OFF + 27]), "+f"(d[OFF + 28]), "+f"(d[OFF + 29]), "+f"(d[OFF + 30]), "+f"(d[OFF + 31]), "+f"(d[OFF + 32]), "+f"(d[OFF + 33]), "+f"(d[OFF + 34]), "+f"(d[OFF + 35]), "+f"(d[OFF + 36]), "+f"(d[OFF + 37]), "+f"(d[OFF + 38]), "+f"(d[OFF + 39]), "+f"(d[OFF + 40]), "+f"(d[OFF + 41]), "+f"(d[OFF + 42]), "+f"(d[OFF + 43]), "+f"(d[OFF + 44]), "+f"(d[OFF + 45]), "+f"(d[OFF + 46]), "+f"(d[OFF + 47]), "+f"(d[OFF + 48]), "+f"(d[OFF + 49]), "+f"(d[OFF + 50]), "+f"(d[OFF + 51]), "+f"(d[OFF + 52]), "+f"(d[OFF + 53]), "+f"(d[OFF + 54]), "+f"(d[OFF + 55]), "+f"(d[OFF + 56]), "+f"(d[OFF + 57]), "+f"(d[OFF + 58]), "+f"(d[OFF + 59]), "+f"(d[OFF + 60]), "+f"(d[OFF + 61]), "+f"(d[OFF + 62]), "+f"(d[OFF + 63]), "+f"(d[OFF + 64]), "+f"(d[OFF + 65]), "+f"(d[OFF + 66]), "+f"(d[OFF + 67]), "+f"(d[OFF + 68]), "+f"(d[OFF + 69]), "+f"(d[OFF + 70]), "+f"(d[OFF + 71]), "+f"(d[OFF + 72]), "+f"(d[OFF + 73]), "+f"(d[OFF + 74]), "+f"(d[OFF + 75]), "+f"(d[OFF + 76]), "+f"(d[OFF + 77]), "+f"(d[OFF + 78]), "+f"(d[OFF + 79]), "+f"(d[OFF + 80]), "+f"(d[OFF + 81]), "+f"(d[OFF + 82]), "+f"(d[OFF + 83]), "+f"(d[OFF + 84]), "+f"(d[OFF + 85]), "+f"(d[OFF + 86]), "+f"(d[OFF + 87]), "+f"(d[OFF + 88]), "+f"(d[OFF + 89]), "+f"(d[OFF + 90]), "+f"(d[OFF + 91]), "+f"(d[OFF + 92]), "+f"(d[OFF + 93]), "+f"(d[OFF + 94]), "+f"(d[OFF + 95]), "+f"(d[OFF + 96]), "+f"(d[OFF + 97]), "+f"(d[OFF + 98]), "+f"(d[OFF + 99]), "+f"(d[OFF + 100]), "+f"(d[OFF + 101]), "+f"(d[OFF + 102]), "+f"(d[OFF + 103]), "+f"(d[OFF + 104]), "+f"(d[OFF + 105]), "+f"(d[OFF + 106]), "+f"(d[OFF + 107]), "+f"(d[OFF + 108]), "+f"(d[OFF + 109]), "+f"(d[OFF + 110]), "+f"(d[OFF + 111]), "+f"(d[OFF + 112]), "+f"(d[OFF + 113]), "+f"(d[OFF + 114]), "+f"(d[OFF + 115]), "+f"(d[OFF + 116]), "+f"(d[OFF + 117]), "+f"(d[OFF + 118]), "+f"(d[OFF + 119]), "+f"(d[OFF + 120]), "+f"(d[OFF + 121]), "+f"(d[OFF + 122]), "+f"(d[OFF + 123]), "+f"(d[OFF + 124]), "+f"(d[OFF + 125]), "+f"(d[OFF + 126]), "+f"(d[OFF + 127])
      : "l"(adesc), "l"(bdesc), "r"(accumulate));
}
__device__ __forceinline__ void wgmma_rs_n128_tb(float (&d)[64], const uint32_t (&a)[4], uint64_t bdesc, uint32_t accumulate) {
  asm volatile(
      "{\n\t.reg .pred p;\n\t"
      "setp.ne.b32 p, %69, 0;\n\t"
      "wgmma.mma_async.sync.aligned.m64n128k16.f32.bf16.bf16 {%0, %1, %2, %3, %4, %5, %6, %7, %8, %9, %10, %11, %12, %13, %14, %15, %16, %17, %18, %19, %20, %21, %22, %23, %24, %25, %26, %27, %28, %29, %30, %31, %32, %33, %34, %35, %36, %37, %38, %39, %40, %41, %42, %43, %44, %45, %46, %47, %48, %49, %50, %51, %52, %53, %54, %55, %56, %57, %58, %59, %60, %61, %62, %63}, {%64, %65, %66, %67}, %68, p, 1, 1, 1;\n\t}\n"
      : "+f"(d[0]), "+f"(d[1]), "+f"(d[2]), "+f"(d[3]), "+f"(d[4]), "+f"(d[5]), "+f"(d[6]), "+f"(d[7]), "+f"(d[8]), "+f"(d[9]), "+f"(d[10]), "+f"(d[11]), "+f"(d[12]), "+f"(d[13]), "+f"(d[14]), "+f"(d[15]), "+f"(d[16]), "+f"(d[17]), "+f"(d[18]), "+f"(d[19]), "+f"(d[20]), "+f"(d[21]), "+f"(d[22]), "+f"(d[23]), "+f"(d[24]), "+f"(d[25]), "+f"(d[26]), "+f"(d[27]), "+f"(d[28]), "+f"(d[29]), "+f"(d[30]), "+f"(d[31]), "+f"(d[32]), "+f"(d[33]), "+f"(d[34]), "+f"(d[35]), "+f"(d[36]), "+f"(d[37]), "+f"(d[38]), "+f"(d[39]), "+f"(d[40]), "+f"(d[41]), "+f"(d[42]), "+f"(d[43]), "+f"(d[44]), "+f"(d[45]), "+f"(d[46]), "+f"(d[47]), "+f"(d[48]), "+f"(d[49]), "+f"(d[50]), "+f"(d[51]), "+f"(d[52]), "+f"(d[53]), "+f"(d[54]), "+f"(d[55]), "+f"(d[56]), "+f"(d[57]), "+f"(d[58]), "+f"(d[59]), "+f"(d[60]), "+f"(d[61]), "+f"(d[62]), "+f"(d[63])
      : "r"(a[0]), "r"(a[1]), "r"(a[2]), "r"(a[3]), "l"(bdesc), "r"(accumulate));
}
template <int TB>
__device__ __forceinline__ void wgmma_ss_acc64(float (&d)[64], uint64_t adesc, uint64_t bdesc, uint32_t accumulate) {
  asm volatile(
      "{\n\t.reg .pred p;\n\t"
      "setp.ne.b32 p, %66, 0;\n\t"
      "wgmma.mma_async.sync.aligned.m64n128k16.f32.bf16.bf16 {%0, %1, %2, %3, %4, %5, %6, %7, %8, %9, %10, %11, %12, %13, %14, %15, %16, %17, %18, %19, %20, %21, %22, %23, %24, %25, %26, %27, %28, %29, %30, %31, %32, %33, %34, %35, %36, %37, %38, %39, %40, %41, %42, %43, %44, %45, %46, %47, %48, %49, %50, %51, %52, %53, %54, %55, %56, %57, %58, %59, %60, %61, %62, %63}, %64, %65, p, 1, 1, 0, %67;\n\t}\n"
      : "+f"(d[0]), "+f"(d[1]), "+f"(d[2]), "+f"(d[3]), "+f"(d[4]), "+f"(d[5]), "+f"(d[6]), "+f"(d[7]), "+f"(d[8]), "+f"(d[9]), "+f"(d[10]), "+f"(d[11]), "+f"(d[12]), "+f"(d[13]), "+f"(d[14]), "+f"(d[15]), "+f"(d[16]), "+f"(d[17]), "+f"(d[18]), "+f"(d[19]), "+f"(d[20]), "+f"(d[21]), "+f"(d[22]), "+f"(d[23]), "+f"(d[24]), "+f"(d[25]), "+f"(d[26]), "+f"(d[27]), "+f"(d[28]), "+f"(d[29]), "+f"(d[30]), "+f"(d[31]), "+f"(d[32]), "+f"(d[33]), "+f"(d[34]), "+f"(d[35]), "+f"(d[36]), "+f"(d[37]), "+f"(d[38]), "+f"(d[39]), "+f"(d[40]), "+f"(d[41]), "+f"(d[42]), "+f"(d[43]), "+f"(d[44]), "+f"(d[45]), "+f"(d[46]), "+f"(d[47]), "+f"(d[48]), "+f"(d[49]), "+f"(d[50]), "+f"(d[51]), "+f"(d[52]), "+f"(d[53]), "+f"(d[54]), "+f"(d[55]), "+f"(d[56]), "+f"(d[57]), "+f"(d[58]), "+f"(d[59]), "+f"(d[60]), "+f"(d[61]), "+f"(d[62]), "+f"(d[63])
      : "l"(adesc), "l"(bdesc), "r"(accumulate), "n"(TB));
}

__device__ __forceinline__ uint32_t pack_bf16x2(float lo, float hi) {
  __nv_bfloat162 v = __floats2bfloat162_rn(lo, hi);
  return *reinterpret_cast<uint32_t*>(&v);
}
__device__ __forceinline__ float fast_exp2(float x) {
  float y;
  asm volatile("ex2.approx.ftz.f32 %0, %1;" : "=f"(y) : "f"(x));
  return y;
}
__device__ __forceinline__ float fast_tanh(float x) {
  float y;
  asm volatile("tanh.approx.f32 %0, %1;" : "=f"(y) : "f"(x));
  return y;
}
__device__ __forceinline__ float gelu_tanh(float x) {
  const float k0 = 0.7978845608028654f, k1 = 0.044715f;
  float u = k0 * (x + k1 * x * x * x);
  return 0.5f * x * (1.0f + fast_tanh(u));
}

}
```

Measured before the change: 41.92.

## Add dual-accumulator N=192 GEMM kernel overlapping epilogue with next tile's MMA

Adds a persistent Hopper GEMM kernel with BLOCK_N=192 in which each consumer warpgroup holds two 96-register accumulators. It runs the previous tile's TMA-store epilogue box by box, interleaved with the first k-blocks of the next tile's wgmma. A planner picks the 192-wide tile for large GEMMs (M>=16384, N>=3072) when it gives fewer wave rounds than 256, which reduces wave quantization. The goal is to hide epilogue time behind MMA and improve tile balance across SMs. The cost is higher register pressure and extra shared-memory epilogue buffers.

```diff
diff --git a/include/yume_b200.h b/include/yume_b200.h
--- a/include/yume_b200.h
+++ b/include/yume_b200.h
@@ -49,6 +49,7 @@
 long long yb_gemm_workspace_bytes(int M, int N, int K, int epilogue, int cta_pair, int split_k);
 int yb_gemm_splitk_plan(int tiles, int num_kb, int clusters, int split_k, int* out3);
 int yb_gemm_plan(int M, int N, int sms, int* out4);
+int yb_gemm_launch_plan(int M, int N, int epilogue, int n_split, int sms, int* out4);
 
 typedef struct yb_conv3d_args {
   unsigned int struct_bytes;
diff --git a/yume_b200/_lib.py b/yume_b200/_lib.py
--- a/yume_b200/_lib.py
+++ b/yume_b200/_lib.py
@@ -61,6 +61,7 @@
     "yb_nchw_to_nhwc_bf16": (_i, [_vp, _vp, _ll, _i, _i, _vp]),
     "yb_nhwc_to_nchw_f32": (_i, [_vp, _ll, _vp, _ll, _i, _vp]),
     "yb_gemm_plan": (_i, [_i, _i, _i, C.POINTER(C.c_int)]),
+    "yb_gemm_launch_plan": (_i, [_i, _i, _i, _i, _i, C.POINTER(C.c_int)]),
     "yb_gemm_workspace_bytes": (_ll, [_i, _i, _i, _i, _i, _i]),
     "yb_gemm_splitk_plan": (_i, [_i, _i, _i, _i, C.POINTER(C.c_int)]),
     "yb_conv3d_plan": (_i, [_i, _i, _i, _i, _i, _i, C.POINTER(C.c_int)]),
diff --git a/yume_b200/csrc/gemm.cu b/yume_b200/csrc/gemm.cu
--- a/yume_b200/csrc/gemm.cu
+++ b/yume_b200/csrc/gemm.cu
@@ -66,12 +66,13 @@
   return s > GEMM_MAX_STAGES ? GEMM_MAX_STAGES : s;
 }
 
+template <int GN = GEMM_GROUP_N>
 __device__ __forceinline__ void tile_coords(int tile, int num_m_tiles, int num_n_tiles, int& m_tile, int& n_tile) {
-  const int per_group = GEMM_GROUP_N * num_m_tiles;
+  const int per_group = GN * num_m_tiles;
   const int g = tile / per_group;
   const int r = tile - g * per_group;
-  const int n_first = g * GEMM_GROUP_N;
-  const int n_in_group = min(GEMM_GROUP_N, num_n_tiles - n_first);
+  const int n_first = g * GN;
+  const int n_in_group = min(GN, num_n_tiles - n_first);
   m_tile = r / n_in_group;
   n_tile = n_first + (r - m_tile * n_in_group);
 }
@@ -190,20 +191,15 @@
   }
 }
 
-template <int EPI, int NM>
-__device__ __forceinline__ void epilogue_tma(const GemmParams& p, const CUtensorMap* tmO, const float (&acc)[128], uint8_t* bufs,
-                                             int row0, int col0, int wg, int wtid, uint32_t& nbox) {
-  constexpr bool kF32 = (EPI == YB_EPI_F32 || EPI == YB_EPI_GATE_RES);
-  constexpr int BOX_COLS = kF32 ? 32 : 64;
-  constexpr int GROUPS = BOX_COLS / 8;
-  if (row0 >= p.M) return;
-  const int lane = wtid & 31;
-  const int r = (wtid >> 5) * 16 + (lane >> 2);
-  const int sw = lane >> 2, c2 = 2 * (lane & 3);
-  const int ncols = min(NM, p.N - col0);
-  const float* g_lo = nullptr;
-  const float* g_hi = nullptr;
+template <int EPI>
+constexpr int epi_box_cols() { return (EPI == YB_EPI_F32 || EPI == YB_EPI_GATE_RES) ? 32 : 64; }
+
+template <int EPI>
+__device__ __forceinline__ void epilogue_gate_rows(const GemmParams& p, int row0, int wtid, const float*& g_lo, const float*& g_hi) {
+  g_lo = nullptr;
+  g_hi = nullptr;
   if (EPI == YB_EPI_GATE_RES && p.gate != nullptr) {
+    const int r = (wtid >> 5) * 16 + ((wtid & 31) >> 2);
     int t_lo = 0, t_hi = 0;
     if (p.tok_idx != nullptr) {
       if (row0 + r < p.M) t_lo = p.tok_idx[row0 + r];
@@ -212,56 +208,77 @@
     g_lo = p.gate + static_cast<long long>(t_lo) * p.gate_ld;
     g_hi = p.gate + static_cast<long long>(t_hi) * p.gate_ld;
   }
-#pragma unroll
-  for (int s = 0; s < NM / BOX_COLS; ++s) {
-    if (s * BOX_COLS < ncols) {
-      uint8_t* buf = bufs + (nbox & 1) * GEMM_EPI_BOX_BYTES;
-      if (wtid == 0) bulk_wait_read<1>();
-      named_bar_sync(1 + wg, 128);
-#pragma unroll
-      for (int j = 0; j < GROUPS; ++j) {
-        const int g = s * GROUPS + j;
-        const int col = col0 + s * BOX_COLS + 8 * j + c2;
-        float2 b = make_float2(0.f, 0.f);
-        const bool in = s * BOX_COLS + 8 * j < ncols;
-        if (p.bias && in) b = __ldg(reinterpret_cast<const float2*>(p.bias + col));
-        float2 lo = make_float2(acc[4 * g] + b.x, acc[4 * g + 1] + b.y);
-        float2 hi = make_float2(acc[4 * g + 2] + b.x, acc[4 * g + 3] + b.y);
-        if (EPI == YB_EPI_GELU_BF16) {
-          lo = make_float2(gelu_tanh(lo.x), gelu_tanh(lo.y));
-          hi = make_float2(gelu_tanh(hi.x), gelu_tanh(hi.y));
-        }
-        if (EPI == YB_EPI_GELU_ERF_BF16) {
-          auto ge = [](float v) { return 0.5f * v * (1.0f + erff(v * 0.7071067811865476f)); };
-          lo = make_float2(ge(lo.x), ge(lo.y));
-          hi = make_float2(ge(hi.x), ge(hi.y));
-        }
-        if (EPI == YB_EPI_GATE_RES && g_lo != nullptr && in) {
-          const float2 gl = __ldg(reinterpret_cast<const float2*>(g_lo + col));
-          const float2 gh = __ldg(reinterpret_cast<const float2*>(g_hi + col));
-          lo = make_float2(lo.x * gl.x, lo.y * gl.y);
-          hi = make_float2(hi.x * gh.x, hi.y * gh.y);
-        }
-        if (kF32) {
-          const int off = (((2 * j + ((lane & 3) >> 1)) ^ sw) << 4) + 8 * (lane & 1);
-          *reinterpret_cast<float2*>(buf + r * 128 + off) = lo;
-          *reinterpret_cast<float2*>(buf + (r + 8) * 128 + off) = hi;
-        } else {
-          const int off = ((j ^ sw) << 4) + 4 * (lane & 3);
-          *reinterpret_cast<uint32_t*>(buf + r * 128 + off) = pack_bf16x2(lo.x, lo.y);
-          *reinterpret_cast<uint32_t*>(buf + (r + 8) * 128 + off) = pack_bf16x2(hi.x, hi.y);
-        }
-      }
-      fence_proxy_async_smem();
-      named_bar_sync(1 + wg, 128);
-      if (wtid == 0) {
-        if (EPI == YB_EPI_GATE_RES) tma_reduce_add_2d(tmO, buf, col0 + s * BOX_COLS, row0);
-        else tma_store_2d(tmO, buf, col0 + s * BOX_COLS, row0);
-        bulk_commit();
-      }
-      ++nbox;
-    }
-  }
+}
+
+template <int EPI, int NBUF, int R>
+__device__ __forceinline__ void epilogue_tma_box(const GemmParams& p, const CUtensorMap* tmO, const float (&acc)[R], uint8_t* bufs,
+                                                 int s, int row0, int col0, int ncols, const float* g_lo, const float* g_hi, int wg,
+                                                 int wtid, uint32_t& nbox) {
+  constexpr bool kF32 = (EPI == YB_EPI_F32 || EPI == YB_EPI_GATE_RES);
+  constexpr int BOX_COLS = epi_box_cols<EPI>();
+  constexpr int GROUPS = BOX_COLS / 8;
+  if (s * BOX_COLS >= ncols) return;
+  const int lane = wtid & 31;
+  const int r = (wtid >> 5) * 16 + (lane >> 2);
+  const int sw = lane >> 2, c2 = 2 * (lane & 3);
+  uint8_t* buf = bufs + (nbox % NBUF) * GEMM_EPI_BOX_BYTES;
+  if (wtid == 0) bulk_wait_read<NBUF - 1>();
+  named_bar_sync(1 + wg, 128);
+#pragma unroll
+  for (int j = 0; j < GROUPS; ++j) {
+    const int g = s * GROUPS + j;
+    const int col = col0 + s * BOX_COLS + 8 * j + c2;
+    float2 b = make_float2(0.f, 0.f);
+    const bool in = s * BOX_COLS + 8 * j < ncols;
+    if (p.bias && in) b = __ldg(reinterpret_cast<const float2*>(p.bias + col));
+    float2 lo = make_float2(acc[4 * g] + b.x, acc[4 * g + 1] + b.y);
+    float2 hi = make_float2(acc[4 * g + 2] + b.x, acc[4 * g + 3] + b.y);
+    if (EPI == YB_EPI_GELU_BF16) {
+      lo = make_float2(gelu_tanh(lo.x), gelu_tanh(lo.y));
+      hi = make_float2(gelu_tanh(hi.x), gelu_tanh(hi.y));
+    }
+    if (EPI == YB_EPI_GELU_ERF_BF16) {
+      auto ge = [](float v) { return 0.5f * v * (1.0f + erff(v * 0.7071067811865476f)); };
+      lo = make_float2(ge(lo.x), ge(lo.y));
+      hi = make_float2(ge(hi.x), ge(hi.y));
+    }
+    if (EPI == YB_EPI_GATE_RES && g_lo != nullptr && in) {
+      const float2 gl = __ldg(reinterpret_cast<const float2*>(g_lo + col));
+      const float2 gh = __ldg(reinterpret_cast<const float2*>(g_hi + col));
+      lo = make_float2(lo.x * gl.x, lo.y * gl.y);
+      hi = make_float2(hi.x * gh.x, hi.y * gh.y);
+    }
+    if (kF32) {
+      const int off = (((2 * j + ((lane & 3) >> 1)) ^ sw) << 4) + 8 * (lane & 1);
+      *reinterpret_cast<float2*>(buf + r * 128 + off) = lo;
+      *reinterpret_cast<float2*>(buf + (r + 8) * 128 + off) = hi;
+    } else {
+      const int off = ((j ^ sw) << 4) + 4 * (lane & 3);
+      *reinterpret_cast<uint32_t*>(buf + r * 128 + off) = pack_bf16x2(lo.x, lo.y);
+      *reinterpret_cast<uint32_t*>(buf + (r + 8) * 128 + off) = pack_bf16x2(hi.x, hi.y);
+    }
+  }
+  fence_proxy_async_smem();
+  named_bar_sync(1 + wg, 128);
+  if (wtid == 0) {
+    if (EPI == YB_EPI_GATE_RES) tma_reduce_add_2d(tmO, buf, col0 + s * BOX_COLS, row0);
+    else tma_store_2d(tmO, buf, col0 + s * BOX_COLS, row0);
+    bulk_commit();
+  }
+  ++nbox;
+}
+
+template <int EPI, int NM, int NBUF = 2, int R>
+__device__ __forceinline__ void epilogue_tma(const GemmParams& p, const CUtensorMap* tmO, const float (&acc)[R], uint8_t* bufs,
+                                             int row0, int col0, int wg, int wtid, uint32_t& nbox) {
+  if (row0 >= p.M) return;
+  const int ncols = min(NM, p.N - col0);
+  const float* g_lo;
+  const float* g_hi;
+  epilogue_gate_rows<EPI>(p, row0, wtid, g_lo, g_hi);
+#pragma unroll
+  for (int s = 0; s < NM / epi_box_cols<EPI>(); ++s)
+    epilogue_tma_box<EPI, NBUF>(p, tmO, acc, bufs, s, row0, col0, ncols, g_lo, g_hi, wg, wtid, nbox);
 }
 
 template <int NM>
@@ -584,6 +601,155 @@
   if (CLUSTER > 1) cluster_sync_all();
 }
 
+constexpr int DUAL_BLOCK_N = 192;
+constexpr int DUAL_STAGES = 4;
+constexpr int DUAL_STAGE_BYTES = GEMM_A_BYTES + gemm_b_bytes(DUAL_BLOCK_N);
+constexpr int DUAL_EPI_BUFS = 4;
+constexpr int DUAL_GROUP_N = 4;
+static_assert(DUAL_STAGES * DUAL_STAGE_BYTES + 2 * DUAL_EPI_BUFS * GEMM_EPI_BOX_BYTES + 1024 + 256 <= GEMM_SMEM_BYTES,
+              "dual GEMM shared memory");
+
+__device__ __forceinline__ void gemm_mma_k64_n192(float (&acc)[96], uint32_t sa, uint32_t sb, bool zero_first) {
+  const uint64_t ad0 = make_smem_desc_sw128(sa, 16, 1024), bd0 = make_smem_desc_sw128(sb, 16, 1024);
+#pragma unroll
+  for (int k = 0; k < GEMM_BLOCK_K / 16; ++k) wgmma_ss_n192(acc, ad0 + 2 * k, bd0 + 2 * k, (zero_first && k == 0) ? 0u : 1u);
+}
+
+struct DualState {
+  int stage, prev;
+  uint32_t phase, nbox;
+  int prow0, pcol0;
+};
+
+template <int EPI>
+__device__ __forceinline__ void dual_tile(const GemmParams& p, const CUtensorMap* tmO, float (&x)[96], float (&y)[96], int tile,
+                                          uint8_t* smem, uint64_t* full_bar, uint64_t* empty_bar, uint8_t* bufs, int wg, int wtid,
+                                          int num_kb, DualState& st) {
+  constexpr int NBOX = DUAL_BLOCK_N / epi_box_cols<EPI>();
+  const int lane = wtid & 31;
+  const bool epi = st.prow0 >= 0 && st.prow0 < p.M;
+  const int ncols = min(DUAL_BLOCK_N, p.N - st.pcol0);
+  const float* g_lo = nullptr;
+  const float* g_hi = nullptr;
+  if (epi) epilogue_gate_rows<EPI>(p, st.prow0, wtid, g_lo, g_hi);
+  auto issue = [&](int kb) {
+    mbar_wait_raised(&full_bar[st.stage], st.phase);
+    const uint32_t sa = smem_u32(smem + st.stage * DUAL_STAGE_BYTES);
+    fence_regs(x);
+    wgmma_fence();
+    gemm_mma_k64_n192(x, sa + wg * 64 * 128, sa + GEMM_A_BYTES, kb == 0);
+    wgmma_commit();
+  };
+  auto retire = [&]() {
+    wgmma_wait<1>();
+    fence_regs(x);
+    if (st.prev >= 0) release_slot<1>(&empty_bar[st.prev], lane);
+    st.prev = st.stage;
+    if (++st.stage == DUAL_STAGES) {
+      st.stage = 0;
+      st.phase ^= 1;
+    }
+  };
+  issue(0);
+  retire();
+  fence_regs(y);
+#pragma unroll
+  for (int s = 1; s <= NBOX; ++s) {
+    if (s < num_kb) issue(s);
+    if (epi) epilogue_tma_box<EPI, DUAL_EPI_BUFS>(p, tmO, y, bufs, s - 1, st.prow0, st.pcol0, ncols, g_lo, g_hi, wg, wtid, st.nbox);
+    if (s < num_kb) retire();
+  }
+#pragma unroll 1
+  for (int kb = NBOX + 1; kb < num_kb; ++kb) {
+    issue(kb);
+    retire();
+  }
+  int m_tile, n_tile;
+  tile_coords<DUAL_GROUP_N>(tile, p.num_m_tiles, p.num_n_tiles, m_tile, n_tile);
+  st.prow0 = m_tile * GEMM_BLOCK_M + wg * 64;
+  st.pcol0 = n_tile * DUAL_BLOCK_N;
+}
+
+template <int EPI>
+__global__ void __launch_bounds__(GEMM_THREADS, 1)
+gemm_dual_kernel(const __grid_constant__ CUtensorMap tmA, const __grid_constant__ CUtensorMap tmB,
+                 const __grid_constant__ CUtensorMap tmO, const GemmParams p) {
+  extern __shared__ uint8_t smem_raw[];
+  uint8_t* smem = reinterpret_cast<uint8_t*>((reinterpret_cast<uintptr_t>(smem_raw) + 1023) & ~uintptr_t(1023));
+  uint8_t* epi_bufs = smem + DUAL_STAGES * DUAL_STAGE_BYTES;
+  uint64_t* full_bar = reinterpret_cast<uint64_t*>(epi_bufs + 2 * DUAL_EPI_BUFS * GEMM_EPI_BOX_BYTES);
+  uint64_t* empty_bar = full_bar + DUAL_STAGES;
+  const int warp = threadIdx.x >> 5, lane = threadIdx.x & 31;
+  const int num_tiles = p.sk_full;
+  const int num_kb = (p.K + GEMM_BLOCK_K - 1) / GEMM_BLOCK_K;
+  if (threadIdx.x == 0) {
+    tma_prefetch_desc(&tmA);
+    tma_prefetch_desc(&tmB);
+    tma_prefetch_desc(&tmO);
+    for (int i = 0; i < DUAL_STAGES; ++i) {
+      mbar_init(&full_bar[i], 1);
+      mbar_init(&empty_bar[i], 8);
+    }
+    fence_barrier_init();
+  }
+  __syncthreads();
+
+  if (warp < 4) {
+    setmaxnreg_dec<24>();
+    if (warp == 0 && lane == 0) {
+      int stage = 0;
+      uint32_t phase = 0;
+      for (int tile = blockIdx.x; tile < num_tiles; tile += gridDim.x) {
+        int m_tile, n_tile;
+        tile_coords<DUAL_GROUP_N>(tile, p.num_m_tiles, p.num_n_tiles, m_tile, n_tile);
+        for (int kb = 0; kb < num_kb; ++kb) {
+          mbar_wait(&empty_bar[stage], phase ^ 1);
+          uint8_t* sa = smem + stage * DUAL_STAGE_BYTES;
+          mbar_arrive_expect_tx(&full_bar[stage], GEMM_A_BYTES + DUAL_BLOCK_N * GEMM_BLOCK_K * 2);
+          const int kcol = kb * GEMM_BLOCK_K;
+          const int chunk = kcol / p.a_split;
+          tma_load_3d(sa, &tmA, &full_bar[stage], kcol - chunk * p.a_split, m_tile * GEMM_BLOCK_M, chunk);
+          tma_load_2d(sa + GEMM_A_BYTES, &tmB, &full_bar[stage], kcol, n_tile * DUAL_BLOCK_N);
+          if (++stage == DUAL_STAGES) {
+            stage = 0;
+            phase ^= 1;
+          }
+        }
+      }
+    }
+  } else {
+    setmaxnreg_inc<240>();
+    const int wg = (warp >> 2) - 1;
+    const int wtid = threadIdx.x & 127;
+    uint8_t* bufs = epi_bufs + wg * DUAL_EPI_BUFS * GEMM_EPI_BOX_BYTES;
+    DualState st = {0, -1, 0u, 0u, -1, 0};
+    float acc0[96], acc1[96];
+#pragma unroll
+    for (int i = 0; i < 96; ++i) {
+      acc0[i] = 0.f;
+      acc1[i] = 0.f;
+    }
+    for (int tile = blockIdx.x; tile < num_tiles; tile += 2 * gridDim.x) {
+      dual_tile<EPI>(p, &tmO, acc0, acc1, tile, smem, full_bar, empty_bar, bufs, wg, wtid, num_kb, st);
+      if (tile + gridDim.x >= num_tiles) {
+        wgmma_wait<0>();
+        fence_regs(acc0);
+        epilogue_tma<EPI, DUAL_BLOCK_N, DUAL_EPI_BUFS>(p, &tmO, acc0, bufs, st.prow0, st.pcol0, wg, wtid, st.nbox);
+        break;
+      }
+      dual_tile<EPI>(p, &tmO, acc1, acc0, tile + gridDim.x, smem, full_bar, empty_bar, bufs, wg, wtid, num_kb, st);
+      if (tile + 2 * gridDim.x >= num_tiles) {
+        wgmma_wait<0>();
+        fence_regs(acc1);
+        epilogue_tma<EPI, DUAL_BLOCK_N, DUAL_EPI_BUFS>(p, &tmO, acc1, bufs, st.prow0, st.pcol0, wg, wtid, st.nbox);
+        break;
+      }
+    }
+    wgmma_wait<0>();
+    if (wtid == 0) bulk_wait<0>();
+  }
+}
+
 __global__ void __launch_bounds__(256) gemm_splitk_combine_kernel(const GemmParams p, int tail_tiles) {
   const int block_n = p.block_n, quads = block_n >> 2;
   const long long total = static_cast<long long>(tail_tiles) * 256 * quads;
@@ -724,6 +890,38 @@
   return check_launch("gemm_splitk_combine");
 }
 
+template <int EPI>
+static int launch_gemm_dual(const CUtensorMap& tmA, const CUtensorMap& tmB, const CUtensorMap& tmO, GemmParams& p,
+                            cudaStream_t stream) {
+  auto kern = gemm_dual_kernel<EPI>;
+  static bool attr_set[kMaxDevices] = {};
+  if (int rc = ensure_dynamic_smem(kern, GEMM_SMEM_BYTES, attr_set, "gemm_dual")) return rc;
+  p.block_n = DUAL_BLOCK_N;
+  p.stages = DUAL_STAGES;
+  p.tma_out = 1;
+  p.num_m_tiles = (p.M + GEMM_BLOCK_M - 1) / GEMM_BLOCK_M;
+  p.num_n_tiles = (p.N + DUAL_BLOCK_N - 1) / DUAL_BLOCK_N;
+  const int tiles = p.num_m_tiles * p.num_n_tiles;
+  p.sk_full = tiles;
+  p.sk_ns = 1;
+  const int grid = tiles < sm_count() ? tiles : sm_count();
+  kern<<<grid, GEMM_THREADS, GEMM_SMEM_BYTES, stream>>>(tmA, tmB, tmO, p);
+  return check_launch("gemm_dual");
+}
+
+static bool gemm_dual_ok(int epilogue, int n_split) {
+  return n_split == 0 && epilogue != YB_EPI_RES_BF16 && epilogue != YB_EPI_GELU_ERF_BF16;
+}
+
+static int gemm_block_n(int M, int N, int sms, bool dual_ok) {
+  const int bn = (N % 256 == 0 || N > 1024) ? 256 : 128;
+  if (!dual_ok || M < 16384 || N < 3072) return bn;
+  const long long m_tiles = (M + GEMM_BLOCK_M - 1) / GEMM_BLOCK_M;
+  const long long rounds256 = (m_tiles * ((N + 255) / 256) + sms - 1) / sms;
+  const long long rounds192 = (m_tiles * ((N + DUAL_BLOCK_N - 1) / DUAL_BLOCK_N) + sms - 1) / sms;
+  return 3 * rounds192 <= 4 * rounds256 ? DUAL_BLOCK_N : bn;
+}
+
 static void conv_plan(int T, int H, int W, int block_n, int kw, int fuse_policy, int* TW, int* TH, int* TT, bool* fused) {
   auto pow2_ge = [](int v) { int p = 1; while (p < v) p <<= 1; return p; };
   double best = -1.0;
@@ -779,7 +977,16 @@
 extern "C" int yb_gemm_plan(int M, int N, int sms, int* out4) {
   if (M <= 0 || N <= 0 || sms < 2 || !out4) return YB_ERR_ARG;
   out4[0] = 0;
-  out4[1] = (N % 256 == 0 || N > 1024) ? 256 : 128;
+  out4[1] = yb::gemm_block_n(M, N, sms, false);
+  out4[2] = (M + yb::GEMM_BLOCK_M - 1) / yb::GEMM_BLOCK_M;
+  out4[3] = (N + out4[1] - 1) / out4[1];
+  return YB_OK;
+}
+
+extern "C" int yb_gemm_launch_plan(int M, int N, int epilogue, int n_split, int sms, int* out4) {
+  if (M <= 0 || N <= 0 || epilogue < 0 || epilogue > YB_EPI_RES_BF16 || n_split < 0 || sms < 2 || !out4) return YB_ERR_ARG;
+  out4[0] = 0;
+  out4[1] = yb::gemm_block_n(M, N, sms, yb::gemm_dual_ok(epilogue, n_split));
   out4[2] = (M + yb::GEMM_BLOCK_M - 1) / yb::GEMM_BLOCK_M;
   out4[3] = (N + out4[1] - 1) / out4[1];
   return YB_OK;
@@ -876,17 +1083,29 @@
       default: return launch_gemm<YB_EPI_GATE_RES, 0, 2>(tmA, tmB, nullptr, p, stream, a->split_k, a->ws, a->ws_bytes);
     }
   }
-  const int block_n = (a->block_n == 128 || a->block_n == 256) ? a->block_n : ((a->N % 256 == 0 || a->N > 1024) ? 256 : 128);
+  const bool tma_epi = a->n_split == 0 && a->epilogue != YB_EPI_RES_BF16;
+  const bool dual_ok = gemm_dual_ok(a->epilogue, a->n_split);
+  if (a->block_n == DUAL_BLOCK_N && !dual_ok) return YB_ERR_ARG;
+  const int block_n = (a->block_n == 128 || a->block_n == DUAL_BLOCK_N || a->block_n == 256)
+                          ? a->block_n : gemm_block_n(a->M, a->N, sm_count(), dual_ok);
   rc = make_tmap_bf16_2d(&tmB, a->B, a->N, a->K, a->ldb, block_n, GEMM_BLOCK_K);
   if (rc) return rc;
   p.block_n = block_n;
   CUtensorMap tmO;
   const CUtensorMap* tmo = nullptr;
-  if (a->n_split == 0 && a->epilogue != YB_EPI_RES_BF16) {
+  if (tma_epi) {
     const int elem = (a->epilogue == YB_EPI_F32 || a->epilogue == YB_EPI_GATE_RES) ? 4 : 2;
     rc = make_tmap_out_2d(&tmO, a->out, a->M, a->N, a->ldo, elem, 64);
     if (rc) return rc;
     tmo = &tmO;
+  }
+  if (block_n == DUAL_BLOCK_N) {
+    switch (a->epilogue) {
+      case YB_EPI_BF16: return launch_gemm_dual<YB_EPI_BF16>(tmA, tmB, tmO, p, stream);
+      case YB_EPI_GELU_BF16: return launch_gemm_dual<YB_EPI_GELU_BF16>(tmA, tmB, tmO, p, stream);
+      case YB_EPI_F32: return launch_gemm_dual<YB_EPI_F32>(tmA, tmB, tmO, p, stream);
+      default: return launch_gemm_dual<YB_EPI_GATE_RES>(tmA, tmB, tmO, p, stream);
+    }
   }
   switch (a->epilogue) {
     case YB_EPI_BF16: return launch_gemm<YB_EPI_BF16, 0, 1>(tmA, tmB, tmo, p, stream);
diff --git a/yume_b200/csrc/yb_ptx.cuh b/yume_b200/csrc/yb_ptx.cuh
--- a/yume_b200/csrc/yb_ptx.cuh
+++ b/yume_b200/csrc/yb_ptx.cuh
@@ -66,6 +66,16 @@
     }
   }
 }
+__device__ __forceinline__ void mbar_wait_raised(uint64_t* bar, uint32_t parity) {
+  if (mbar_try_wait(bar, parity)) return;
+  const long long t0 = clock64();
+  while (!mbar_try_wait(bar, parity)) {
+    if (clock64() - t0 > YB_WAIT_LIMIT_CYCLES) {
+      asm volatile("trap;");
+      break;
+    }
+  }
+}
 __device__ __forceinline__ void mbar_wait_cluster(uint64_t* bar, uint32_t parity) {
   const long long t0 = clock64();
   for (;;) {
@@ -195,6 +205,14 @@
       : "+f"(d[OFF + 0]), "+f"(d[OFF + 1]), "+f"(d[OFF + 2]), "+f"(d[OFF + 3]), "+f"(d[OFF + 4]), "+f"(d[OFF + 5]), "+f"(d[OFF + 6]), "+f"(d[OFF + 7]), "+f"(d[OFF + 8]), "+f"(d[OFF + 9]), "+f"(d[OFF + 10]), "+f"(d[OFF + 11]), "+f"(d[OFF + 12]), "+f"(d[OFF + 13]), "+f"(d[OFF + 14]), "+f"(d[OFF + 15]), "+f"(d[OFF + 16]), "+f"(d[OFF + 17]), "+f"(d[OFF + 18]), "+f"(d[OFF + 19]), "+f"(d[OFF + 20]), "+f"(d[OFF + 21]), "+f"(d[OFF + 22]), "+f"(d[OFF + 23]), "+f"(d[OFF + 24]), "+f"(d[OFF + 25]), "+f"(d[OFF + 26]), "+f"(d[OFF + 27]), "+f"(d[OFF + 28]), "+f"(d[OFF + 29]), "+f"(d[OFF + 30]), "+f"(d[OFF + 31]), "+f"(d[OFF + 32]), "+f"(d[OFF + 33]), "+f"(d[OFF + 34]), "+f"(d[OFF + 35]), "+f"(d[OFF + 36]), "+f"(d[OFF + 37]), "+f"(d[OFF + 38]), "+f"(d[OFF + 39]), "+f"(d[OFF + 40]), "+f"(d[OFF + 41]), "+f"(d[OFF + 42]), "+f"(d[OFF + 43]), "+f"(d[OFF + 44]), "+f"(d[OFF + 45]), "+f"(d[OFF + 46]), "+f"(d[OFF + 47]), "+f"(d[OFF + 48]), "+f"(d[OFF + 49]), "+f"(d[OFF + 50]), "+f"(d[OFF + 51]), "+f"(d[OFF + 52]), "+f"(d[OFF + 53]), "+f"(d[OFF + 54]), "+f"(d[OFF + 55]), "+f"(d[OFF + 56]), "+f"(d[OFF + 57]), "+f"(d[OFF + 58]), "+f"(d[OFF + 59]), "+f"(d[OFF + 60]), "+f"(d[OFF + 61]), "+f"(d[OFF + 62]), "+f"(d[OFF + 63]), "+f"(d[OFF + 64]), "+f"(d[OFF + 65]), "+f"(d[OFF + 66]), "+f"(d[OFF + 67]), "+f"(d[OFF + 68]), "+f"(d[OFF + 69]), "+f"(d[OFF + 70]), "+f"(d[OFF + 71]), "+f"(d[OFF + 72]), "+f"(d[OFF + 73]), "+f"(d[OFF + 74]), "+f"(d[OFF + 75]), "+f"(d[OFF + 76]), "+f"(d[OFF + 77]), "+f"(d[OFF + 78]), "+f"(d[OFF + 79]), "+f"(d[OFF + 80]), "+f"(d[OFF + 81]), "+f"(d[OFF + 82]), "+f"(d[OFF + 83]), "+f"(d[OFF + 84]), "+f"(d[OFF + 85]), "+f"(d[OFF + 86]), "+f"(d[OFF + 87]), "+f"(d[OFF + 88]), "+f"(d[OFF + 89]), "+f"(d[OFF + 90]), "+f"(d[OFF + 91]), "+f"(d[OFF + 92]), "+f"(d[OFF + 93]), "+f"(d[OFF + 94]), "+f"(d[OFF + 95]), "+f"(d[OFF + 96]), "+f"(d[OFF + 97]), "+f"(d[OFF + 98]), "+f"(d[OFF + 99]), "+f"(d[OFF + 100]), "+f"(d[OFF + 101]), "+f"(d[OFF + 102]), "+f"(d[OFF + 103]), "+f"(d[OFF + 104]), "+f"(d[OFF + 105]), "+f"(d[OFF + 106]), "+f"(d[OFF + 107]), "+f"(d[OFF + 108]), "+f"(d[OFF + 109]), "+f"(d[OFF + 110]), "+f"(d[OFF + 111]), "+f"(d[OFF + 112]), "+f"(d[OFF + 113]), "+f"(d[OFF + 114]), "+f"(d[OFF + 115]), "+f"(d[OFF + 116]), "+f"(d[OFF + 117]), "+f"(d[OFF + 118]), "+f"(d[OFF + 119]), "+f"(d[OFF + 120]), "+f"(d[OFF + 121]), "+f"(d[OFF + 122]), "+f"(d[OFF + 123]), "+f"(d[OFF + 124]), "+f"(d[OFF + 125]), "+f"(d[OFF + 126]), "+f"(d[OFF + 127])
       : "l"(adesc), "l"(bdesc), "r"(accumulate));
 }
+__device__ __forceinline__ void wgmma_ss_n192(float (&d)[96], uint64_t adesc, uint64_t bdesc, uint32_t accumulate) {
+  asm volatile(
+      "{\n\t.reg .pred p;\n\t"
+      "setp.ne.b32 p, %98, 0;\n\t"
+      "wgmma.mma_async.sync.aligned.m64n192k16.f32.bf16.bf16 {%0, %1, %2, %3, %4, %5, %6, %7, %8, %9, %10, %11, %12, %13, %14, %15, %16, %17, %18, %19, %20, %21, %22, %23, %24, %25, %26, %27, %28, %29, %30, %31, %32, %33, %34, %35, %36, %37, %38, %39, %40, %41, %42, %43, %44, %45, %46, %47, %48, %49, %50, %51, %52, %53, %54, %55, %56, %57, %58, %59, %60, %61, %62, %63, %64, %65, %66, %67, %68, %69, %70, %71, %72, %73, %74, %75, %76, %77, %78, %79, %80, %81, %82, %83, %84, %85, %86, %87, %88, %89, %90, %91, %92, %93, %94, %95}, %96, %97, p, 1, 1, 0, 0;\n\t}\n"
+      : "+f"(d[0]), "+f"(d[1]), "+f"(d[2]), "+f"(d[3]), "+f"(d[4]), "+f"(d[5]), "+f"(d[6]), "+f"(d[7]), "+f"(d[8]), "+f"(d[9]), "+f"(d[10]), "+f"(d[11]), "+f"(d[12]), "+f"(d[13]), "+f"(d[14]), "+f"(d[15]), "+f"(d[16]), "+f"(d[17]), "+f"(d[18]), "+f"(d[19]), "+f"(d[20]), "+f"(d[21]), "+f"(d[22]), "+f"(d[23]), "+f"(d[24]), "+f"(d[25]), "+f"(d[26]), "+f"(d[27]), "+f"(d[28]), "+f"(d[29]), "+f"(d[30]), "+f"(d[31]), "+f"(d[32]), "+f"(d[33]), "+f"(d[34]), "+f"(d[35]), "+f"(d[36]), "+f"(d[37]), "+f"(d[38]), "+f"(d[39]), "+f"(d[40]), "+f"(d[41]), "+f"(d[42]), "+f"(d[43]), "+f"(d[44]), "+f"(d[45]), "+f"(d[46]), "+f"(d[47]), "+f"(d[48]), "+f"(d[49]), "+f"(d[50]), "+f"(d[51]), "+f"(d[52]), "+f"(d[53]), "+f"(d[54]), "+f"(d[55]), "+f"(d[56]), "+f"(d[57]), "+f"(d[58]), "+f"(d[59]), "+f"(d[60]), "+f"(d[61]), "+f"(d[62]), "+f"(d[63]), "+f"(d[64]), "+f"(d[65]), "+f"(d[66]), "+f"(d[67]), "+f"(d[68]), "+f"(d[69]), "+f"(d[70]), "+f"(d[71]), "+f"(d[72]), "+f"(d[73]), "+f"(d[74]), "+f"(d[75]), "+f"(d[76]), "+f"(d[77]), "+f"(d[78]), "+f"(d[79]), "+f"(d[80]), "+f"(d[81]), "+f"(d[82]), "+f"(d[83]), "+f"(d[84]), "+f"(d[85]), "+f"(d[86]), "+f"(d[87]), "+f"(d[88]), "+f"(d[89]), "+f"(d[90]), "+f"(d[91]), "+f"(d[92]), "+f"(d[93]), "+f"(d[94]), "+f"(d[95])
+      : "l"(adesc), "l"(bdesc), "r"(accumulate));
+}
 __device__ __forceinline__ void wgmma_rs_n128_tb(float (&d)[64], const uint32_t (&a)[4], uint64_t bdesc, uint32_t accumulate) {
   asm volatile(
       "{\n\t.reg .pred p;\n\t"
```

New measurement: 42.04, median of 6. About the same (+0.3%).
